# automerge/automerge-classic

Measured on AMD Instinct MI355X. Metric: CRDT ops/sec applied (bulk replay), higher is better.
Workload: dtype u32

## Files before the change

### automerge_classic_amd/csrc/am355_api.hip

```cpp
#include "am355_ctx.h"
#include "am355_scan.h"
#include "am355_textrec.h"

static bool ctx_init(am355_ctx* c) {
  {
    unsigned hw = std::thread::hardware_concurrency();
    const char* env = getenv("AM355_HOST_THREADS");
    unsigned want = env && atoi(env) > 0 ? (unsigned)atoi(env) : std::min(hw ? hw : 4u, 64u);
    c->pool.reset(new HostPool(want > 1 ? want - 1 : 0));
  }
  int prio_low = 0, prio_high = 0;
  (void)hipDeviceGetStreamPriorityRange(&prio_low, &prio_high);
  auto make_stream = [](Stream& s, int prio) { return hipStreamCreateWithPriority(&s.h, hipStreamNonBlocking, prio) == hipSuccess; };
  if (!make_stream(c->stream, prio_high)) return false;
  {
    const char* env = getenv("AM355_HASH_CUS");
    int want = env ? atoi(env) : 0;
    bool made = false;
    if (want > 0) {
      hipDeviceProp_t prop;
      if (hipGetDeviceProperties(&prop, c->device) == hipSuccess && prop.multiProcessorCount > want) {
        int n_cu = prop.multiProcessorCount;
        std::vector<uint32_t> mask((size_t)(n_cu + 31) / 32, 0u);
        for (int k = 0; k < want; k++) { int cu = n_cu - 1 - k; mask[(size_t)cu / 32] |= 1u << (cu % 32); }
// ... 9 lines not shown
  if (!c->h_sig.ensure(sizeof(HostSignals))) return false;
  memset(c->h_sig.p, 0, sizeof(HostSignals));
  if (const char* e = getenv("AM355_PHASE_EVENTS")) c->phase_events = strcmp(e, "0") != 0;
  return true;
}

extern "C" am355_ctx* am355_create(int device) {
  int n = 0;
  if (hipGetDeviceCount(&n) != hipSuccess || n <= 0 || device < 0 || device >= n) return nullptr;
  (void)hipSetDeviceFlags(hipDeviceScheduleSpin);
  if (hipSetDevice(device) != hipSuccess) return nullptr;
  am355_ctx* c = new am355_ctx();
  c->device = device;
  if (!ctx_init(c)) { delete c; return nullptr; }
  return c;
}

am355_ctx::~am355_ctx() {
  (void)hipSetDevice(device);
  if (lane) lane->wait();
  (void)doc_sum.wait();
  for (const Stream* s : {&stream, &stream2, &stream3, &stream4})
    if (s->h) (void)hipStreamSynchronize(s->h);
  if (shard_comm) (void)am355_shard_finalize(this);
}

extern "C" void am355_destroy(am355_ctx* c) {
  delete c;
}

extern "C" const char* am355_last_error(const am355_ctx* c) { return c ? c->err.c_str() : "no context (no GPU?)"; }
extern "C" uint32_t am355_flags(const am355_ctx* c) { return c ? c->flags : 0; }

extern "C" int am355_set_phase_events(am355_ctx* c, int on) {
  if (!c) return AM355_E_ARG;
  c->phase_events = on != 0;
  return AM355_OK;
}

extern "C" int am355_get_stats(const am355_ctx* c, am355_stats* out) {
  if (!c || !out) return AM355_E_ARG;
  *out = c->stats;
  return AM355_OK;
}

extern "C" int am355_get_hashes(const am355_ctx* c, uint8_t* out) {
  if (!c || !out) return AM355_E_ARG;
  if (!c->replayed || !c->h_hashes.p || c->is_document) return AM355_E_STATE;
  memcpy(out, c->h_hashes.p, 32 * (size_t)c->n_changes);
  return AM355_OK;
}

extern "C" int am355_arena_epoch(const am355_ctx* c, uint64_t* epoch) {
  if (!c || !epoch) return AM355_E_ARG;
  *epoch = c->arena_epoch;
  return AM355_OK;
}

extern "C" int am355_get_hashes_range(const am355_ctx* c, uint32_t first, uint32_t count, uint8_t* out) {
  if (!c || (!out && count)) return AM355_E_ARG;
  if (!c->replayed || !c->h_hashes.p || c->is_document) return AM355_E_STATE;
  if (first > c->n_changes || count > c->n_changes - first) return AM355_E_ARG;
  if (count) memcpy(out, (const uint8_t*)c->h_hashes.p + 32 * (size_t)first, 32 * (size_t)count);
  return AM355_OK;
}

extern "C" int am355_applied_in_input_order(const am355_ctx* c, int* yes) {
  if (!c || !yes) return AM355_E_ARG;
  if (!c->replayed || c->is_document) return AM355_E_STATE;
  bool ok = c->pending_change.empty() && c->n_pending == 0 && c->applied_change.size() == c->n_changes;
  for (uint32_t i = 0; ok && i < c->n_changes; i++) ok = c->applied_change[i] == i;
  *yes = ok ? 1 : 0;
  return AM355_OK;
}

extern "C" int am355_resident_counters(const am355_ctx* c, uint64_t out[3]) {
  if (!c || !out) return AM355_E_ARG;
  out[0] = c->n_resident_calls;
  out[1] = c->n_resident_fallbacks;
  out[2] = c->n_resorder_calls;
  return AM355_OK;
}

extern "C" int am355_resident_maps_only_calls(const am355_ctx* c, uint64_t* out) {
  if (!c || !out) return AM355_E_ARG;
  *out = c->n_maps_only_calls;
  return AM355_OK;
}

extern "C" int am355_set_resident_new_actors(am355_ctx* c, int on) {
  if (!c) return AM355_E_ARG;
  c->resident_new_actors = on != 0;
  return AM355_OK;
}

extern "C" int am355_resident_new_actor_calls(const am355_ctx* c, uint64_t out[2]) {
  if (!c || !out) return AM355_E_ARG;
  out[0] = c->n_new_actor_calls;
  out[1] = c->n_rank_rewrites;
  return AM355_OK;
}

extern "C" int am355_set_resident_map_merge(am355_ctx* c, int on) {
  if (!c) return AM355_E_ARG;
  c->resident_map_merge = on != 0;
  return AM355_OK;
}

extern "C" int am355_resident_map_merge_calls(const am355_ctx* c, uint64_t out[2]) {
  if (!c || !out) return AM355_E_ARG;
  out[0] = c->n_map_merge_calls;
  out[1] = c->n_map_merge_declined;
  return AM355_OK;
}

extern "C" int am355_set_resident_new_objects(am355_ctx* c, int on) {
  if (!c) return AM355_E_ARG;
  c->resident_new_objects = on != 0;
  return AM355_OK;
}

extern "C" int am355_resident_new_object_calls(const am355_ctx* c, uint64_t out[2]) {
  if (!c || !out) return AM355_E_ARG;
  out[0] = c->n_new_object_calls;
  out[1] = c->n_new_object_declined;
  return AM355_OK;
}

extern "C" int am355_set_resident_counters(am355_ctx* c, int on) {
  if (!c) return AM355_E_ARG;
  c->resident_counters = on != 0;
  return AM355_OK;
}

extern "C" int am355_set_local_small(am355_ctx* c, int on) {
  if (!c) return AM355_E_ARG;
  c->local_small = on != 0;
  return AM355_OK;
}

extern "C" int am355_local_small_calls(const am355_ctx* c, uint64_t out[2]) {
  if (!c || !out) return AM355_E_ARG;
  out[0] = c->n_local_small;
  out[1] = c->n_local_small_bulk;
  return AM355_OK;
}

extern "C" int am355_resident_counter_calls(const am355_ctx* c, uint64_t out[2]) {
  if (!c || !out) return AM355_E_ARG;
  out[0] = c->n_counter_calls;
  out[1] = c->n_counter_declined;
  return AM355_OK;
}

extern "C" int am355_get_raw(const am355_ctx* c, const uint8_t** arena, const uint64_t** offsets, uint32_t* n) {
  if (!c || !c->staged) return AM355_E_STATE;
  if (arena) *arena = c->raw.data();
  if (offsets) *offsets = c->raw_off.data();
  if (n) *n = c->n_changes;
  return AM355_OK;
}

extern "C" int am355_get_applied(const am355_ctx* c, uint32_t* out, uint32_t* n_applied) {
  if (!c || !n_applied) return AM355_E_ARG;
  if (!c->replayed || c->is_document) return AM355_E_STATE;
  *n_applied = (uint32_t)c->applied_change.size();
// ... 393 lines not shown
```

### automerge_classic_amd/csrc/am355_ctx.h

```cpp
#pragma once
#include "../../include/am355.h"
#include "am355_decode.h"
#include "am355_merge.h"
#include "am355_bigcol.h"
#include "am355_encode.h"
#include "am355_prims.h"
#include "am355_render.h"
#include "am355_host.h"
#include "am355_pinflate.h"
#include "am355_history.h"
#include "am355_delta.h"
#include "am355_resorder.h"
#include "am355_apply.h"
#include "am355_sync.h"
#include "am355_sched.h"
#include "am355_hist.h"
#include "am355_canary.h"

#include <zlib.h>

#include <algorithm>
#include <atomic>
#include <chrono>
#include <cstdarg>
// ... 310 lines not shown
  std::vector<uint64_t> raw_off;
  uint32_t n_changes = 0;
  DevBuf d_plan_totals;
  bool spec_launched = false;
  bool spec_large_launched = false;
  uint32_t spec_cap_ops = 0, spec_cap_preds = 0;
  uint32_t hint_ops = 0, hint_preds = 0, hint_large = 0;
  bool staged = false, replayed = false, ir_fetched = false;
  int ir_copy_enqueued = 0;
  bool prefetch_ir = false;
  bool has_unknown_cols = false;
  bool staging_in_flight = false;
  bool is_document = false;
  ChangeMeta doc_meta{};
  std::vector<uint32_t> doc_actor_rank;
  DevBuf d_arena, d_offsets, d_metas;
  uint64_t arena_epoch = 1;
  CopyRanges pending_up;
  std::vector<uint32_t> breaks_dev;
  void* breaks_dev_ptr = nullptr;
  HostBuf h_breaks_ahead;
  bool offsets_on_device = false;
  HostBuf h_metas, h_offsets, h_sig;
  uint32_t sig_seq = 0;
  Event ev_s1;
  Event ev_fills;
  Event ev_sched;
  Event ev_plan, ev_tables;
  void* counts_zeroed_at = nullptr; size_t counts_zeroed = 0;
  bool phase_events = false;
  DevBuf d_big, d_bigvals, d_ks;
  HostBuf h_biginfo;
  BigColDesc doc_cols{};
  bool doc_serial = false;
  DevBuf d_entries, d_amap_base, d_amap_prov, d_slots, d_first_idx, d_hashes, d_hash_tab, d_min_idx, d_has_dep, d_words, d_slot_rank, d_scan1, d_plan_sums, d_dep_idx, d_self_idx, d_rank_ids;
  HostBuf h_dep_idx, h_self_idx, h_amap, h_amap_base;
  HostBuf h_slots, h_hashes, h_has_dep, h_words, h_stage, h_s1;
  DevBuf d_s1;
  ChangeBrief* hp_briefs = nullptr;
  uint32_t* hp_distinct = nullptr;
  bool have_host_metas = false;
  uint32_t amap_cap = 0, slot_mask = 0, hash_mask = 0;
  bool used_fast_path = false;

  std::vector<ChangePlan> plans;
  std::vector<uint32_t> applied_change, applied_op_base;
  struct DocSum {
    static constexpr size_t PIECE = (size_t)4 << 20;
    std::thread t;
    std::unique_ptr<std::atomic<uint8_t>[]> copied;
    size_t n_pieces = 0;
    bool pending = false, ok = false;
    bool wait() {
      if (t.joinable()) t.join();
      pending = false;
      return ok;
    }
    ~DocSum() { if (t.joinable()) t.join(); }
  } doc_sum;
  std::vector<uint8_t> doc_bytes;
  std::vector<uint8_t> saved;
  HistoryOutput history;
  bool history_ok = false; uint32_t history_flags = 0;
  std::vector<std::vector<uint8_t>> inflate_scratch;
  std::vector<std::unique_ptr<PInflateJob>> pinflate_jobs;
  std::vector<uint32_t> doc_col_rows;
  std::vector<std::pair<uint32_t, std::vector<uint8_t>>> doc_chg_cols;
  std::vector<uint8_t> doc_tail;
  bool doc_other_ops_cols = false;
  DevBuf d_save, d_enc, d_encout;
  HostBuf h_encout;
  std::vector<uint32_t> amap;
  std::vector<ActorSpan> spans;
  std::vector<uint32_t> actor_tab_off;
  std::vector<std::string> actors;
  std::vector<uint32_t> clock_actor;
  std::vector<uint64_t> clock_seq;
  std::vector<uint8_t> heads;
  uint32_t n_applied = 0, n_pending = 0;
  uint64_t n_ops = 0, n_preds = 0, max_op = 0;
  DevBuf d_plans, d_amap, d_tables;
  ActorSpan* p_spans = nullptr;
  uint32_t* p_tab_off = nullptr;

  DevBuf d_cols, d_pred, d_merge, d_sort, d_ir, d_counts;
  OpCols cols{};
  MergeBufs mb{};
  PatchIR ir{};
  HostBuf h_counts;
  Counts counts{};

  HostBuf h_ir, h_rows;
  am355_patch_ir hir{};
  std::vector<uint32_t> actor_off;
  std::vector<uint8_t> actor_bytes;
  std::string json;

  am355_stats stats{};

  std::vector<uint32_t> pending_change;
  std::vector<uint32_t> pass_first_row;
  DevBuf d_delta, d_pass, d_delta_edit, d_sched, d_hist;
  HostBuf h_sched;
  bool key_unbounded = false;
  bool device_scheduled = false;
  HostBuf h_delta;
  DeltaBufs delta{};
  bool h_tables_current = false, h_tables_were_current = false;
  bool batch_list_only = false;
  void* apply_tail = nullptr;
  ApplyPatch apply;
  bool apply_ready = false;
  std::vector<uint32_t> dep_first, dep_index;
  bool dep_graph_ready = false;
  DevBuf d_sync;
  struct GraphIndex {
    uint64_t epoch = ~0ull;
    uint32_t n_staged = 0, n_applied = 0;
    std::vector<uint32_t> dep_first, dep_index;
    std::vector<uint8_t> is_applied;
    std::vector<uint32_t> table;
    std::vector<uint32_t> dpt_first, dpt_index;
    uint32_t dpt_applied = 0;
    std::vector<uint32_t> chain_head, chain_tail, chain_child, chain_next;
    std::vector<uint32_t> out_idx;
    std::vector<uint8_t> out_hashes;
    std::vector<uint64_t> absent;
    uint64_t tab_epoch = ~0ull;
    uint32_t tab_n = 0, tab_mask = 0;
  } graph;
  uint64_t graph_epoch = 0;
  uint32_t graph_probe_min = 65536;
  uint64_t n_graph_device = 0, n_graph_host = 0;
  DevBuf d_graph;
  HostBuf h_graph;
  std::vector<uint32_t> stream_breaks;
  bool breaks_exact = true, children_hazard = false, in_apply = false;
  uint32_t graph_mode = 0, doc_n_changes = 0, sched_prefix = 0;
  bool doc_head_index_known = true, sched_graph_after = true;
  bool doc_graph_known = false;
  uint64_t doc_rows = 0;
  bool doc_rows_known = false;
  bool no_history = false;
  DevBuf d_breaks;
  HostBuf h_delta_tabs;
  bool state_checked = false;
  std::string apply_json;

  struct Keep { bool want = false; uint32_t n_changes = 0; uint64_t n_ops = 0, n_preds = 0; } keep;
  uint32_t cols_cap_ops = 0, cols_cap_preds = 0;
  bool resident_valid = false;
  struct ResidentMark { uint32_t lost[8] = {}; uint32_t n_changes = 0; uint64_t n_ops = 0, n_preds = 0; } res_mark;
  uint32_t seed_list_inc = 0;
  std::vector<uint32_t> hash_index;
  uint32_t hash_index_n = 0;
  std::vector<uint32_t> res_rank_of;
  uint32_t res_rank_n = 0;
  struct ActorMemo { std::vector<uint8_t> bytes; std::vector<uint32_t> ranks; };
  std::vector<ActorMemo> res_actor_memo;
  DevBuf d_pos, d_order_alt, d_resorder;
  uint32_t* order_alt_ptr = nullptr;
  HostBuf h_resorder;
  bool pos_valid = false;
  bool ir_stale = false;
  uint64_t n_resorder_calls = 0;
  uint64_t n_maps_only_calls = 0;
// ... 148 lines not shown
```

### automerge_classic_amd/csrc/am355_decode.h

```cpp
#pragma once
#include "am355_internal.h"

namespace am355 {
struct ParseFills {
  uint32_t* p[5];
  uint64_t n_words[5];
  uint32_t value[5];
  uint32_t n;
};
void parse_changes_host(const uint8_t* arena, const uint64_t* offsets, uint32_t n_changes, ChangeMeta* metas, uint32_t* n_entries);
void launch_parse_changes(const uint8_t* arena, const uint64_t* offsets, uint32_t n_changes, ChangeMeta* metas, uint32_t* n_entries, const ParseFills& fills,
                          hipStream_t st, bool fat = false);
int change_wave_class(const ChangeMeta& m);
void launch_hash_changes(const uint8_t* arena, const uint64_t* offsets, uint32_t n, uint8_t* hashes, uint32_t* min_idx, uint32_t* hash_tab,
                         uint32_t tab_mask, uint32_t* flags, hipStream_t st);
void launch_deps_resolve(const uint8_t* arena, const ChangeMeta* metas, const uint8_t* hashes, uint32_t n, const uint32_t* hash_tab, uint32_t tab_mask,
                         const uint32_t* min_idx, uint8_t* has_dependent, uint32_t* fast_flags, uint32_t* dep_idx, uint32_t* self_idx, hipStream_t st);
void launch_actor_intern(const uint8_t* arena, ChangeMeta* metas, uint32_t n, const uint32_t* amap_base, uint32_t* amap, uint32_t amap_cap,
                         unsigned long long* slots, uint32_t slot_mask, uint32_t* first_idx, uint32_t* flags, uint32_t* fast_flags, uint32_t* distinct,
                         void* rank_ids, ChangeBrief* briefs, uint32_t* slot_rank, unsigned long long* block_sums, uint32_t* plan_words, hipStream_t st,
                         ChangeBrief* host_briefs = nullptr);
size_t rank_ids_bytes();
size_t plan_block_sums_bytes(uint32_t n);
uint32_t distinct_capacity();
void launch_plan(const ChangeBrief* briefs, uint32_t n, const uint32_t* distinct, const uint32_t* slot_rank, uint32_t slot_mask, const unsigned long long* block_sums,
                 ChangePlan* plans, ChangePlan* plans_serial, const uint32_t* words, const uint32_t* plan_words, HostSignals* sig, uint32_t seq, hipStream_t st,
                 PlanTotals* dev_totals = nullptr, uint32_t* host_s1 = nullptr);
void launch_decode_speculative(const uint8_t* arena, const ChangeMeta* metas, const ChangePlan* plans, uint32_t n_changes, const PlanTotals* totals, uint32_t cap_ops,
                               uint32_t cap_preds, uint32_t cap_distinct, const uint32_t* amap, const uint32_t* slot_rank, OpCols cols, uint32_t* flags, hipStream_t st,
                               hipStream_t aux, bool with_large, uint32_t shard_rank = 0, uint32_t shard_world = 1);
void launch_decode_planned(const uint8_t* arena, const ChangeMeta* metas, const ChangePlan* plans, const ChangePlan* plans_serial, uint32_t n_changes,
                           uint32_t n_small, uint32_t n_large, uint32_t n_serial, const uint32_t* amap, const uint32_t* slot_rank, OpCols cols, uint32_t* flags,
                           hipStream_t st, hipStream_t aux, uint32_t shard_rank = 0, uint32_t shard_world = 1);
void launch_decode_columns(const uint8_t* arena, const ChangeMeta* metas, const ChangePlan* plans, uint32_t n_small, uint32_t n_large, uint32_t n_serial,
                           const uint32_t* amap, const uint32_t* slot_rank, OpCols cols, uint32_t* flags, hipStream_t st, hipStream_t aux, uint32_t shard_rank = 0,
                           uint32_t shard_world = 1);
void launch_doc_count(const uint8_t* arena, ChangeMeta* meta, hipStream_t st);
void launch_decode_document(const uint8_t* arena, const ChangeMeta* meta, const ChangePlan* plan, const uint32_t* actor_rank, OpCols cols,
                            uint32_t* flags, hipStream_t st);
void launch_keystr_expand(const uint32_t* run_start, const uint32_t* run_off, const uint32_t* run_len, const uint32_t* n_runs, uint32_t n_rows,
                          uint32_t* key_off, uint32_t* key_len, hipStream_t st);
}
```

### automerge_classic_amd/csrc/am355_decode.hip

```cpp
#include "am355_decode.h"
#include "am355_scan.h"

#include <cstdlib>

namespace am355 {

struct __attribute__((packed)) U8B {
  uint64_t v;
};
__host__ __device__ __forceinline__ uint64_t load_u64_unaligned(const uint8_t* p) { return ((const U8B*)p)->v; }
#ifdef AM355_LDS_IS_DISTINCT
__device__ __forceinline__ uint64_t load_u64_unaligned(LdsBytes p) { return ((const __attribute__((address_space(3))) U8B*)p)->v; }
#endif

template <class P>
struct CurT {
  P p;
  uint32_t off, len;
  uint64_t win;
  uint32_t win_off;
  __host__ __device__ __forceinline__ CurT() {}
  static constexpr uint32_t WIN_EMPTY = 0xffffff00u;
  __host__ __device__ __forceinline__ CurT(P p_, uint32_t off_, uint32_t len_) : p(p_), off(off_), len(len_), win(0), win_off(WIN_EMPTY) {}
  __host__ __device__ __forceinline__ uint32_t byte_at(uint32_t o) {
// ... 987 lines not shown
  __syncthreads();
  ex[0] = ba + ia - a; ex[1] = bb + ib - b; ex[2] = bc + ic - c;
  t[0] = ta; t[1] = tb; t[2] = tc;
}

__device__ void rank_actors(const uint32_t* __restrict__ distinct, const RankId* __restrict__ rank_ids, uint32_t* __restrict__ slot_rank,
                            uint32_t* __restrict__ plan_words) {
  __shared__ unsigned long long s_id[PLAN_RANK_MAX][PLAN_ID_MAX / 8];
  __shared__ uint32_t s_len[PLAN_RANK_MAX];
  __shared__ uint32_t s_fallback;
  static_assert(PLAN_RANK_MAX % BLOCK == 0 && PLAN_RANK_MAX <= DISTINCT_CAP, "rank_actors: records per thread");
  constexpr uint32_t PER = PLAN_RANK_MAX / BLOCK;
  const uint32_t t = threadIdx.x;
  RankId rec[PER];
  uint32_t slot_of[PER];
#pragma unroll
  for (uint32_t k = 0; k < PER; k++) {
    rec[k] = rank_ids[t + k * BLOCK];
    slot_of[k] = distinct[1 + t + k * BLOCK];
  }
  const uint32_t nd = distinct[0];
  if (t == 0) s_fallback = nd > PLAN_RANK_MAX ? 1u : 0u;
  __syncthreads();
  if (nd <= PLAN_RANK_MAX) {
#pragma unroll
    for (uint32_t k = 0; k < PER; k++) {
      const uint32_t a = t + k * BLOCK;
      if (a < nd) {
        s_len[a] = rec[k].len;
        if (rec[k].len > PLAN_ID_MAX) s_fallback = 1;
        for (uint32_t wd = 0; wd < PLAN_ID_MAX / 8; wd++) s_id[a][wd] = rec[k].w[wd];
      }
    }
  }
  __syncthreads();
  if (s_fallback) { if (t == 0) plan_words[0] = 1; return; }
#pragma unroll
  for (uint32_t k = 0; k < PER; k++) {
    const uint32_t a = t + k * BLOCK;
    if (a >= nd) break;
    uint32_t rank = 0;
    const uint32_t my_len = rec[k].len;
    static_assert(PLAN_ID_MAX == 32, "rank_actors compares four 64-bit words");
    const unsigned long long m0 = rec[k].w[0], m1 = rec[k].w[1], m2 = rec[k].w[2], m3 = rec[k].w[3];
    for (uint32_t j = 0; j < nd; j++) {
      const unsigned long long x0 = s_id[j][0], x1 = s_id[j][1], x2 = s_id[j][2], x3 = s_id[j][3];
      const bool less = x0 != m0 ? x0 < m0 : x1 != m1 ? x1 < m1 : x2 != m2 ? x2 < m2 : x3 != m3 ? x3 < m3 : s_len[j] < my_len;
      rank += less ? 1u : 0u;
    }
    slot_rank[slot_of[k]] = rank;
  }
}

__global__ __launch_bounds__(WAVE) void k_actor_first(ChangeMeta* __restrict__ metas, uint32_t n, const uint32_t* __restrict__ amap_base,
                                                       const uint32_t* __restrict__ amap, uint32_t amap_cap, const uint32_t* __restrict__ first_idx,
                                                       uint32_t* __restrict__ fast_flags) {
  wave_priority_high();
  uint32_t c = blockIdx.x, lane = threadIdx.x;
  if (c >= n) return;
  ChangeMeta* m = &metas[c];
  if (m->flags) return;
  uint32_t base = amap_base[c], ne = m->n_entries;
  if ((uint64_t)base + ne > amap_cap) return;
  uint32_t mx = 0;
  for (uint32_t k = lane; k < ne; k += WAVE) {
    uint32_t f = first_idx[amap[base + k]];
    mx = f > mx ? f : mx;
  }
  for (int d = WAVE / 2; d >= 1; d >>= 1) {
    uint32_t o = __shfl_xor(mx, d);
    mx = o > mx ? o : mx;
  }
  if (lane == 0) {
    m->max_first = mx;
    if (mx > c) atomicOr(fast_flags, (uint32_t)FF_LATE_ACTOR);
  }
}

__global__ __launch_bounds__(BLOCK) void k_actor_check(const uint8_t* __restrict__ arena, ChangeMeta* __restrict__ metas, uint32_t n,
                                                       const uint32_t* __restrict__ amap_base, const uint32_t* __restrict__ amap, uint32_t amap_cap,
                                                       const uint32_t* __restrict__ first_idx, uint32_t* __restrict__ flags, uint32_t* __restrict__ fast_flags,
                                                       ChangeBrief* __restrict__ briefs, const uint32_t* __restrict__ distinct, const RankId* __restrict__ rank_ids,
                                                       uint32_t* __restrict__ slot_rank, unsigned long long* __restrict__ block_sums, uint32_t* __restrict__ plan_words,
                                                       ChangeBrief* __restrict__ host_briefs) {
  wave_priority_high();
  __shared__ unsigned long long s_scan[BLOCK / WAVE][3];
  if (blockIdx.x + 1 == gridDim.x) {
    rank_actors(distinct, rank_ids, slot_rank, plan_words);
    return;
  }
  uint32_t c = gtid();
  const bool in_range = c < n;
  ChangeBrief br{};
  if (in_range) {
    ChangeMeta* m = &metas[c];
    br.seq = m->seq;
    br.start_op = (uint32_t)m->start_op;
    br.n_ops = m->n_ops;
    br.n_preds = m->n_preds;
    br.n_entries = m->n_entries;
    br.author_slot = m->author_slot;
    br.flags_fits = m->flags;
    if (!m->flags) {
      int wc = wave_class_of(*m);
      if (wc >= 1) br.flags_fits |= 0x80000000u;
      if (wc == 2) br.flags_fits |= 0x40000000u;
      if (m->pad & 1) br.flags_fits |= 0x20000000u;
    }
    briefs[c] = br;
    if (host_briefs) host_briefs[c] = br;
  }
  const bool valid = in_range && !(br.flags_fits & 0x1fffffffu);
  const bool has = valid && br.n_ops != 0;
  const bool small = has && (br.flags_fits & 0x40000000u), large = has && !small && (br.flags_fits & 0x80000000u), serial = has && !small && !large;
  unsigned long long ex[3], t1[3], t2[3];
  block_scan3(valid ? br.n_ops : 0u, valid ? br.n_preds : 0u, valid ? br.n_entries : 0u, s_scan, ex, t1);
  block_scan3(small ? 1u : 0u, large ? 1u : 0u, serial ? 1u : 0u, s_scan, ex, t2);
  uint32_t mx_op = has ? br.start_op + br.n_ops - 1 : 0u, bad = in_range ? (br.flags_fits & 0x1fffffffu) : 0u, unknown = in_range ? (br.flags_fits & 0x20000000u) : 0u;
  for (int d = WAVE / 2; d >= 1; d >>= 1) {
    uint32_t o = __shfl_xor(mx_op, d), ob = __shfl_xor(bad, d), ou = __shfl_xor(unknown, d);
    mx_op = o > mx_op ? o : mx_op;
    bad |= ob;
    unknown |= ou;
  }
  if ((threadIdx.x & (WAVE - 1)) == 0) {
    if (mx_op) atomicMax(&plan_words[1], mx_op);
    if (bad) atomicOr(&plan_words[2], bad);
    if (unknown) atomicOr(&plan_words[3], 1u);
  }
  if (threadIdx.x == 0) {
    unsigned long long* out = block_sums + (size_t)blockIdx.x * PLAN_SUMS;
    out[0] = t1[0]; out[1] = t1[1]; out[2] = t1[2]; out[3] = t2[0]; out[4] = t2[1]; out[5] = t2[2];
  }
}

__global__ __launch_bounds__(BLOCK) void k_plan_apply(const ChangeBrief* __restrict__ briefs, uint32_t n, const uint32_t* __restrict__ slot_rank, uint32_t slot_mask,
                                                      const unsigned long long* __restrict__ block_sums, ChangePlan* __restrict__ plans,
                                                      ChangePlan* __restrict__ plans_serial, const uint32_t* __restrict__ words, const uint32_t* __restrict__ plan_words,
                                                      const uint32_t* __restrict__ distinct, HostSignals* sig, uint32_t seq, PlanTotals* __restrict__ dev_totals,
                                                      uint32_t* __restrict__ host_s1) {
  wave_priority_high();
  __shared__ unsigned long long s_scan[BLOCK / WAVE][3];
  __shared__ unsigned long long s_base[6];
  {
    unsigned long long p0 = 0, p1 = 0, p2 = 0, p3 = 0, p4 = 0, p5 = 0;
    for (uint32_t j = threadIdx.x; j < blockIdx.x; j += BLOCK) {
      const unsigned long long* q = block_sums + (size_t)j * PLAN_SUMS;
      p0 += q[0]; p1 += q[1]; p2 += q[2]; p3 += q[3]; p4 += q[4]; p5 += q[5];
    }
    unsigned long long ex[3], t1[3], t2[3];
    block_scan3(p0, p1, p2, s_scan, ex, t1);
    block_scan3(p3, p4, p5, s_scan, ex, t2);
    if (threadIdx.x == 0) { s_base[0] = t1[0]; s_base[1] = t1[1]; s_base[2] = t1[2]; s_base[3] = t2[0]; s_base[4] = t2[1]; s_base[5] = t2[2]; }
    __syncthreads();
  }
  const uint32_t c = gtid();
  const bool in_range = c < n;
  ChangeBrief br{};
  if (in_range) br = briefs[c];
  const bool valid = in_range && !(br.flags_fits & 0x1fffffffu);
  const bool has = valid && br.n_ops != 0;
  const bool small = has && (br.flags_fits & 0x40000000u), large = has && !small && (br.flags_fits & 0x80000000u), serial = has && !small && !large;
  unsigned long long e1[3], e2[3], t1[3], t2[3];
  block_scan3(valid ? br.n_ops : 0u, valid ? br.n_preds : 0u, valid ? br.n_entries : 0u, s_scan, e1, t1);
  block_scan3(small ? 1u : 0u, large ? 1u : 0u, serial ? 1u : 0u, s_scan, e2, t2);
  if (has) {
    ChangePlan pl{c, (uint32_t)(s_base[0] + e1[0]), (uint32_t)(s_base[1] + e1[1]), (uint32_t)(s_base[2] + e1[2]),
                  br.author_slot <= slot_mask ? slot_rank[br.author_slot] : 0u, br.n_entries};
    if (small) plans[(uint32_t)(s_base[3] + e2[0])] = pl;
    else if (large) plans[n - 1 - (uint32_t)(s_base[4] + e2[1])] = pl;
    else plans_serial[(uint32_t)(s_base[5] + e2[2])] = pl;
  }
  if (blockIdx.x + 1 == gridDim.x && host_s1) {
    const uint32_t nd = distinct[0] < DISTINCT_CAP ? distinct[0] : DISTINCT_CAP;
    const uint32_t* src = words;
    for (uint32_t i = threadIdx.x; i < 16; i += BLOCK) host_s1[i] = src[i];
    uint32_t* hd = host_s1 + 16;
    for (uint32_t i = threadIdx.x; i < 1 + nd; i += BLOCK) hd[i] = distinct[i];
    const unsigned long long* ids = (const unsigned long long*)(distinct + 2 + DISTINCT_CAP);
    unsigned long long* hids = (unsigned long long*)(hd + 2 + DISTINCT_CAP);
    for (uint32_t i = threadIdx.x; i < nd; i += BLOCK) hids[i] = ids[i];
    __threadfence_system();
    __syncthreads();
  }
  if (blockIdx.x + 1 == gridDim.x && threadIdx.x == 0) {
    unsigned long long ops = s_base[0] + t1[0], preds = s_base[1] + t1[1], ent = s_base[2] + t1[2];
    PlanTotals z{};
    z.n_ops = (uint32_t)ops; z.n_preds = (uint32_t)preds; z.n_entries = (uint32_t)ent;
    z.n_small = (uint32_t)(s_base[3] + t2[0]); z.n_large = (uint32_t)(s_base[4] + t2[1]); z.n_serial = (uint32_t)(s_base[5] + t2[2]);
    z.max_op = plan_words[1];
    z.fallback = (plan_words[0] || ops >= 0x7ffffff0ull || preds >= 0xfffffff0ull || ent >= 0xfffffff0ull) ? 1u : 0u;
    z.flags_a = words[0] | plan_words[2]; z.fast_a = words[1]; z.total_entries = words[2]; z.n_distinct = distinct[0];
    z.reserved[0] = plan_words[3];
    if (dev_totals) *dev_totals = z;
    signal_host((uint32_t*)&sig->plan, (const uint32_t*)&z, sizeof(PlanTotals) / 4, &sig->plan_seq, seq);
  }
}

struct Rle {
  Cur c;
  int state;
  int64_t count;
  bool have_last, last_null;
  int64_t last;
  uint32_t last_off, last_len;
};

__device__ __forceinline__ void rle_init(Rle& r, const uint8_t* p, uint32_t len) {
  r.c = Cur(p, 0, len);
  r.state = 0;
  r.count = 0;
  r.have_last = false;
  r.last_null = true;
  r.last = 0;
  r.last_off = r.last_len = 0;
}

enum { RT_UINT = 0, RT_INT = 1, RT_UTF8 = 2 };

struct RVal {
  bool is_null;
  int64_t i;
  uint32_t off, len;
};

template <int TYPE>
__device__ __forceinline__ bool rle_raw(Rle& r, RVal& v) {
  v.is_null = false;
  if (TYPE == RT_UINT) {
    uint64_t u;
    if (!read_uleb(r.c, u)) return false;
    v.i = (int64_t)u;
  } else if (TYPE == RT_INT) {
    if (!read_sleb(r.c, v.i)) return false;
  } else {
    uint64_t n;
    if (!read_uleb(r.c, n)) return false;
    v.off = r.c.off;
    v.len = (uint32_t)n;
    if (!skip_bytes(r.c, n)) return false;
  }
  return true;
}

template <int TYPE>
__device__ __forceinline__ bool rle_same(const Rle& r, const RVal& v) {
  if (!r.have_last || r.last_null) return false;
  if (TYPE == RT_UTF8) {
    return r.last_len == v.len && bytes_equal(r.c.p, r.last_off, v.off, v.len, r.c.len);
  }
  return r.last == v.i;
}

template <int TYPE>
__device__ __forceinline__ void rle_set_last(Rle& r, const RVal& v) {
  r.have_last = true;
  r.last_null = v.is_null;
  r.last = v.i;
  r.last_off = v.off;
  r.last_len = v.len;
}

template <int TYPE>
__device__ bool rle_next(Rle& r, RVal& v) {
  if (r.count == 0 && r.c.off >= r.c.len) {
    v.is_null = true;
    v.i = 0;
    v.off = v.len = 0;
    return true;
  }
  if (r.count == 0) {
    int64_t n;
    if (!read_sleb(r.c, n)) return false;
    if (n > 1) {
      RVal x;
      x.off = x.len = 0;
// ... 853 lines not shown
      }
    }
  }
  }
  if (groups & DG_PRED) {
  uint32_t total_preds = 0;
  load_col(C_PRED_NUM);
  err |= L.err;
  {
    int64_t carry = 0;
    for (uint32_t i0 = 0; i0 < n; i0 += WAVE) {
      uint32_t i = i0 + lane;
      bool nul = true; int64_t k = 0;
      if (i < n) wv_row_value<false>(L, i, nul, k, err);
      if (nul) k = 0;
      int64_t incl = carry + wave_incl_scan_i64(k, lane);
      carry = __shfl(incl, WAVE - 1);
      if (i < n) {
        if ((uint64_t)incl > n_preds_cap) { err |= F_BAD_RLE; k = 0; incl = 0; }
        o.pred_num[base + i] = (uint32_t)k;
        o.pred_first[base + i] = pl.pred_base + (uint32_t)(incl - k);
      }
    }
    total_preds = (uint64_t)carry > n_preds_cap ? 0 : (uint32_t)carry;
  }
  load_col(C_PRED_ACTOR);
  err |= L.err;
  for (uint32_t j = lane; j < total_preds; j += WAVE) {
    bool nul; int64_t v;
    wv_row_value<false>(L, j, nul, v, err);
    uint32_t r = 0;
    if (nul) err |= F_UNSUPPORTED;
    else if ((uint64_t)v >= pl.n_actors) err |= F_BAD_ROW;
    else r = L.rank[v];
    o.pred_actor[pl.pred_base + j] = r;
  }
  load_col(C_PRED_CTR);
  err |= L.err;
  {
    int64_t carry = 0;
    for (uint32_t j0 = 0; j0 < total_preds; j0 += WAVE) {
      uint32_t j = j0 + lane;
      bool nul = true; int64_t d = 0;
      if (j < total_preds) wv_row_value<true>(L, j, nul, d, err);
      int64_t abs = carry + wave_incl_scan_i64(nul ? 0 : d, lane);
      carry = __shfl(abs, WAVE - 1);
      if (j < total_preds) {
        if (nul) err |= F_UNSUPPORTED;
        else if (abs < 0 || (uint64_t)abs >= NONE32) err |= F_OVERFLOW;
        o.pred_ctr[pl.pred_base + j] = (uint32_t)abs;
      }
    }
  }
  }
  if (err) atomicOr(flags, err);
}

int change_wave_class(const ChangeMeta& m) { return wave_class_of(m); }

void launch_parse_changes(const uint8_t* arena, const uint64_t* offsets, uint32_t n_changes, ChangeMeta* metas, uint32_t* n_entries, const ParseFills& fills,
                          hipStream_t st, bool fat) {
  if (!n_changes && !fills.n) return;
  if (fat) hipLaunchKernelGGL(k_parse_changes<true>, dim3(n_changes ? n_changes : 64), dim3(WAVE), 0, st, arena, offsets, n_changes, metas, n_entries, fills);
  else hipLaunchKernelGGL(k_parse_changes<false>, dim3(n_changes ? n_changes : 64), dim3(WAVE), 0, st, arena, offsets, n_changes, metas, n_entries, fills);
}

void launch_hash_changes(const uint8_t* arena, const uint64_t* offsets, uint32_t n, uint8_t* hashes, uint32_t* min_idx, uint32_t* hash_tab,
                         uint32_t tab_mask, uint32_t* flags, hipStream_t st) {
  if (!n) return;
  hipLaunchKernelGGL(k_hash_changes, dim3((n + HASH_LANES - 1) / HASH_LANES), dim3(2 * HASH_LANES), 0, st, arena, offsets, n, hashes, min_idx, flags);
  AM355_LAUNCH_INDEPENDENT(k_hash_insert, dim3((n + BLOCK - 1) / BLOCK), dim3(BLOCK), st, (const uint8_t*)hashes, n, hash_tab, tab_mask, min_idx);
}

void launch_deps_resolve(const uint8_t* arena, const ChangeMeta* metas, const uint8_t* hashes, uint32_t n, const uint32_t* hash_tab, uint32_t tab_mask,
                         const uint32_t* min_idx, uint8_t* has_dependent, uint32_t* fast_flags, uint32_t* dep_idx, uint32_t* self_idx, hipStream_t st) {
  if (!n) return;
  AM355_LAUNCH_INDEPENDENT(k_deps_resolve, dim3(n), dim3(WAVE), st, arena, metas, hashes, n, hash_tab, tab_mask, min_idx, has_dependent, fast_flags, dep_idx,
                           self_idx);
}

void launch_actor_intern(const uint8_t* arena, ChangeMeta* metas, uint32_t n, const uint32_t* amap_base, uint32_t* amap, uint32_t amap_cap,
                         unsigned long long* slots, uint32_t slot_mask, uint32_t* first_idx, uint32_t* flags, uint32_t* fast_flags, uint32_t* distinct,
                         void* rank_ids, ChangeBrief* briefs, uint32_t* slot_rank, unsigned long long* block_sums, uint32_t* plan_words, hipStream_t st,
                         ChangeBrief* host_briefs) {
  if (n)
    hipLaunchKernelGGL(k_actor_intern, dim3(n), dim3(WAVE), 0, st, arena, metas, n, amap_base, amap, amap_cap, slots, slot_mask, first_idx, flags,
                       fast_flags, distinct, (RankId*)rank_ids);
  if (n) hipLaunchKernelGGL(k_actor_first, dim3(n), dim3(WAVE), 0, st, metas, n, amap_base, (const uint32_t*)amap, amap_cap, (const uint32_t*)first_idx, fast_flags);
  hipLaunchKernelGGL(k_actor_check, dim3((n + BLOCK - 1) / BLOCK + 1), dim3(BLOCK), 0, st, arena, metas, n, amap_base, (const uint32_t*)amap, amap_cap,
                     (const uint32_t*)first_idx, flags, fast_flags, briefs, (const uint32_t*)distinct, (const RankId*)rank_ids, slot_rank, block_sums, plan_words,
                     host_briefs);
}

size_t rank_ids_bytes() { return sizeof(RankId) * PLAN_RANK_MAX; }

size_t plan_block_sums_bytes(uint32_t n) { return sizeof(unsigned long long) * PLAN_SUMS * ((size_t)(n + BLOCK - 1) / BLOCK + 1); }

void launch_plan(const ChangeBrief* briefs, uint32_t n, const uint32_t* distinct, const uint32_t* slot_rank, uint32_t slot_mask, const unsigned long long* block_sums,
                 ChangePlan* plans, ChangePlan* plans_serial, const uint32_t* words, const uint32_t* plan_words, HostSignals* sig, uint32_t seq, hipStream_t st,
                 PlanTotals* dev_totals, uint32_t* host_s1) {
  uint32_t nb = (n + BLOCK - 1) / BLOCK;
  hipLaunchKernelGGL(k_plan_apply, dim3(nb ? nb : 1), dim3(BLOCK), 0, st, briefs, n, slot_rank, slot_mask, block_sums, plans, plans_serial, words, plan_words,
                     distinct, sig, seq, dev_totals, host_s1);
}

uint32_t distinct_capacity() { return DISTINCT_CAP; }

__global__ __launch_bounds__(WAVE) void k_doc_count(const uint8_t* __restrict__ arena, ChangeMeta* __restrict__ meta) {
  uint32_t lane = threadIdx.x;
  if (lane > 1) return;
  int slot = lane == 0 ? C_ACTION : C_PRED_NUM;
  uint64_t cnt, sum;
  bool ok = rle_count_sum(arena + meta->base + meta->col_off[slot], meta->col_len[slot], cnt, sum);
  if (!ok) { atomicOr(&meta->flags, (uint32_t)F_BAD_RLE); return; }
  if (lane == 0) meta->n_ops = (uint32_t)cnt; else meta->n_preds = (uint32_t)sum;
}

void launch_doc_count(const uint8_t* arena, ChangeMeta* meta, hipStream_t st) {
  AM355_LAUNCH_INDEPENDENT(k_doc_count, dim3(1), dim3(WAVE), st, arena, meta);
}

__global__ __launch_bounds__(BLOCK) void k_keystr_expand(const uint32_t* __restrict__ run_start, const uint32_t* __restrict__ run_off,
                                                          const uint32_t* __restrict__ run_len, const uint32_t* __restrict__ n_runs_p, uint32_t n_rows,
                                                          uint32_t* __restrict__ key_off, uint32_t* __restrict__ key_len) {
  uint32_t row = gtid();
  if (row >= n_rows) return;
  uint32_t nr = *n_runs_p;
  uint32_t off = 0, len = NONE32;
  if (nr && row < run_start[nr]) {
    uint32_t lo = 0, hi = nr;
    while (hi - lo > 1) {
      uint32_t mid = (lo + hi) >> 1;
      if (run_start[mid] <= row) lo = mid; else hi = mid;
    }
    off = run_off[lo];
    len = run_len[lo];
  }
  key_off[row] = off;
  key_len[row] = len;
}

void launch_keystr_expand(const uint32_t* run_start, const uint32_t* run_off, const uint32_t* run_len, const uint32_t* n_runs, uint32_t n_rows,
                          uint32_t* key_off, uint32_t* key_len, hipStream_t st) {
  if (!n_rows) return;
  AM355_LAUNCH_INDEPENDENT(k_keystr_expand, dim3((n_rows + BLOCK - 1) / BLOCK), dim3(BLOCK), st, run_start, run_off, run_len, n_runs, n_rows, key_off, key_len);
}

void launch_decode_document(const uint8_t* arena, const ChangeMeta* meta, const ChangePlan* plan, const uint32_t* actor_rank, OpCols cols,
                            uint32_t* flags, hipStream_t st) {
  ActorXlate x{actor_rank, nullptr, 0, 1};
  AM355_LAUNCH_INDEPENDENT(k_decode_columns, dim3(1, T_NUM_DOC), dim3(WAVE), st, arena, meta, plan, 1u, x, cols, flags, 0);
}

static uint32_t decode_group_split(uint32_t n_waves, uint32_t shard_world, bool large_class = false) {
  static const uint32_t split_max = []() { const char* e = getenv("AM355_DECODE_SPLIT_MAX"); return e && atol(e) > 0 ? (uint32_t)atol(e) : 1536u; }();
  return (shard_world <= 1 && n_waves <= (large_class ? 512u : split_max)) ? 4u : 1u;
}

void launch_decode_columns(const uint8_t* arena, const ChangeMeta* metas, const ChangePlan* plans, uint32_t n_small, uint32_t n_large, uint32_t n_serial,
                           const uint32_t* amap, const uint32_t* slot_rank, OpCols cols, uint32_t* flags, hipStream_t st, hipStream_t aux, uint32_t shard_rank,
                           uint32_t shard_world) {
  ActorXlate x{amap, slot_rank, shard_rank, shard_world};
  if (n_large && n_small + n_large <= 1024) { n_large += n_small; n_small = 0; }
  hipStream_t s2 = (n_small && aux) ? aux : st;
  if (n_small) hipLaunchKernelGGL(k_decode_wave<WaveLdsSmall>, dim3(n_small, decode_group_split(n_small, shard_world)), dim3(WAVE), 0, st, arena, metas, plans, n_small, x, cols, flags, DecodeGate{});
  if (n_large) hipLaunchKernelGGL(k_decode_wave<WaveLdsLarge>, dim3(n_large, decode_group_split(n_large, shard_world, true)), dim3(WAVE), 0, s2, arena, metas, plans + n_small, n_large, x, cols, flags, DecodeGate{});
  if (n_serial)
    AM355_LAUNCH_INDEPENDENT(k_decode_columns, dim3((n_serial + WAVE - 1) / WAVE, T_NUM), dim3(WAVE), s2, arena, metas, plans + n_small + n_large, n_serial,
                             x, cols, flags, 0);
}

void launch_decode_planned(const uint8_t* arena, const ChangeMeta* metas, const ChangePlan* plans, const ChangePlan* plans_serial, uint32_t n_changes,
                           uint32_t n_small, uint32_t n_large, uint32_t n_serial, const uint32_t* amap, const uint32_t* slot_rank, OpCols cols, uint32_t* flags,
                           hipStream_t st, hipStream_t aux, uint32_t shard_rank, uint32_t shard_world) {
  ActorXlate x{amap, slot_rank, shard_rank, shard_world};
  hipStream_t s2 = (n_small && aux) ? aux : st;
  if (n_small) hipLaunchKernelGGL(k_decode_wave<WaveLdsSmall>, dim3(n_small, decode_group_split(n_small, shard_world)), dim3(WAVE), 0, st, arena, metas, plans, n_small, x, cols, flags, DecodeGate{});
  if (n_large) hipLaunchKernelGGL(k_decode_wave<WaveLdsLarge>, dim3(n_large, decode_group_split(n_large, shard_world, true)), dim3(WAVE), 0, s2, arena, metas, plans + (n_changes - n_large), n_large, x, cols, flags, DecodeGate{});
  if (n_serial)
    AM355_LAUNCH_INDEPENDENT(k_decode_columns, dim3((n_serial + WAVE - 1) / WAVE, T_NUM), dim3(WAVE), s2, arena, metas, plans_serial, n_serial, x, cols, flags, 0);
}

void launch_decode_speculative(const uint8_t* arena, const ChangeMeta* metas, const ChangePlan* plans, uint32_t n_changes, const PlanTotals* totals, uint32_t cap_ops,
                               uint32_t cap_preds, uint32_t cap_distinct, const uint32_t* amap, const uint32_t* slot_rank, OpCols cols, uint32_t* flags, hipStream_t st,
                               hipStream_t aux, bool with_large, uint32_t shard_rank, uint32_t shard_world) {
  if (!n_changes) return;
  ActorXlate x{amap, slot_rank, shard_rank, shard_world};
  hipLaunchKernelGGL(k_decode_wave<WaveLdsSmall>, dim3(n_changes, decode_group_split(n_changes, shard_world)), dim3(WAVE), 0, st, arena, metas, plans, 0u, x, cols, flags,
                     DecodeGate{totals, cap_ops, cap_preds, cap_distinct, n_changes, 0u});
// ... 7 lines not shown
```

### automerge_classic_amd/csrc/am355_replay.hip

```cpp
#include "am355_ctx.h"


template <class IsHead>
static void set_heads(am355_ctx* c, uint32_t n, IsHead is_head) {
  std::vector<const uint8_t*> hs;
  for (uint32_t i = 0; i < n; i++)
    if (is_head(i)) hs.push_back(c->h_hashes.as<uint8_t>() + 32 * (size_t)i);
  std::sort(hs.begin(), hs.end(), [](const uint8_t* x, const uint8_t* y) { return memcmp(x, y, 32) < 0; });
  c->heads.resize(hs.size() * 32);
  for (size_t i = 0; i < hs.size(); i++) memcpy(&c->heads[32 * i], hs[i], 32);
}

template <class SpanOf>
static int build_actor_spans(am355_ctx* c, uint32_t na, std::vector<uint32_t>& cnt, SpanOf span_of) {
  c->actor_tab_off.assign(na + 1, 0);
  for (uint32_t a = 0; a < na; a++) c->actor_tab_off[a + 1] = c->actor_tab_off[a] + cnt[a];
  c->spans.resize(c->actor_tab_off[na]);
  for (uint32_t a = 0; a < na; a++) cnt[a] = c->actor_tab_off[a];
  for (const ChangePlan& pl : c->plans) { ActorSpan s = span_of(pl); s.op_base = pl.op_base; c->spans[cnt[pl.author]++] = s; }
  for (uint32_t a = 0; a < na; a++) {
    ActorSpan* v = c->spans.data() + c->actor_tab_off[a];
    size_t k_n = c->actor_tab_off[a + 1] - c->actor_tab_off[a];
    bool sorted = true;
    for (size_t k = 1; k < k_n; k++) sorted = sorted && v[k - 1].start_op <= v[k].start_op;
    if (!sorted) std::sort(v, v + k_n, [](const ActorSpan& x, const ActorSpan& y) { return x.start_op < y.start_op; });
    for (size_t k = 1; k < k_n; k++)
      if ((uint64_t)v[k - 1].start_op + v[k - 1].n_ops > v[k].start_op) {
        c->flags |= AM355_F_DUP_OPID;
        return fail(c, AM355_E_INVALID, "overlapping op id ranges for one actor (duplicate operation ID)");
      }
  }
  return AM355_OK;
}

static constexpr uint32_t UNSET = 0xffffffffu, NEVER = 0xfffffffeu, BUSY = 0xfffffffdu;

struct LineageInput {
  uint32_t n, na, na0, nd;
  bool doc_head_index_known;
  const ChangeMeta* metas;
  const uint32_t *self, *dep_idx, *dep_first, *dep_count, *rank, *local_ids, *local_off;
  std::vector<uint8_t> doc_has_dependent;
};
struct LineageOutcome { std::vector<uint32_t> pass, gpass, gpos; bool graph_after = true; uint32_t flags = 0; };
static LineageOutcome schedule_lineage(const LineageInput& in, bool graph_known) {
  const uint32_t n = in.n, na0 = in.na0, nd = in.nd;
  const ChangeMeta* metas = in.metas;
  LineageOutcome o;
  auto author_of = [&](uint32_t ci) { return in.rank[in.local_ids[in.local_off[ci]]]; };
  auto group_of = [&](uint32_t ci) { return in.self[ci] < n ? in.self[ci] : ci; };
  o.pass.assign(n, NEVER); o.gpass.assign(n, NEVER); o.gpos.assign(n, 0);
  std::vector<uint8_t> vis_dep(n, 0), vis_dup(n, 0), in_round(n, 0);
  std::vector<uint64_t> clk(in.na, 0);
  for (uint32_t i = 0; i < na0; i++) { clk[author_of(i)] = metas[i].seq; o.pass[i] = 0; o.gpass[group_of(i)] = 0; o.gpos[group_of(i)] = i; }
  auto all_prior = [&]() {
    std::fill(vis_dep.begin(), vis_dep.end(), 0); std::fill(vis_dup.begin(), vis_dup.end(), 0);
    for (uint32_t i = 0; i < na0; i++) vis_dep[group_of(i)] = vis_dup[group_of(i)] = 1;
  };
  if (graph_known) all_prior();
  else {
    for (uint32_t i = nd; i < na0; i++) vis_dep[group_of(i)] = vis_dup[group_of(i)] = 1;
    for (uint32_t i = 0; i < nd; i++)
      if (!in.doc_has_dependent[i]) { vis_dup[i] = 1; vis_dep[i] = in.doc_head_index_known ? 1 : 0; }
  }
  std::vector<uint32_t> queue, app, enq;
  for (uint32_t ci = na0; ci < n; ci++) queue.push_back(ci);
  bool graph = graph_known;
  uint32_t round_pass = 0;
  while (!queue.empty()) {
    app.clear(); enq.clear();
    std::vector<uint64_t> clk2 = clk;
    bool aborted = false;
    for (uint32_t ci : queue) {
      const uint32_t F = group_of(ci);
      if (vis_dup[F] || in_round[F]) continue;
      bool ready = true;
      for (uint32_t k = 0; k < in.dep_count[ci] && ready; k++) { const uint32_t dd = in.dep_idx[in.dep_first[ci] + k]; ready = dd < n && (vis_dep[dd] || in_round[dd]); }
      const uint32_t a = author_of(ci);
      const uint64_t expected = clk2[a] + 1;
      if (!ready) enq.push_back(ci);
      else if (metas[ci].seq < expected) {
        if (graph) { o.flags |= AM355_F_BAD_SEQ; return o; }
        aborted = true;
        break;
      } else if (metas[ci].seq > expected) { o.flags |= AM355_F_BAD_SEQ; return o; }
      else { clk2[a] = metas[ci].seq; in_round[F] = 1; app.push_back(ci); }
    }
    for (uint32_t ci : app) in_round[group_of(ci)] = 0;
    if (aborted) { app.clear(); enq = queue; }
    if (!app.empty()) {
      for (uint32_t ci : app) { const uint32_t F = group_of(ci); o.pass[ci] = round_pass; o.gpass[F] = round_pass; o.gpos[F] = ci; vis_dep[F] = vis_dup[F] = 1; }
      clk = clk2;
      round_pass++;
    }
    queue = enq;
    if (queue.empty()) break;
    if (app.empty()) {
      if (graph) break;
      graph = true;
      all_prior();
    }
  }
  o.graph_after = graph;
  return o;
}

static uint32_t rank_device_actors(am355_ctx* c, std::vector<uint32_t>& slot_rank);
// ... 195 lines not shown
  uint64_t ops = 0, preds = 0, max_op = 0;
  std::vector<uint32_t> span_cnt(na + 1, 0);
  c->applied_change.clear();
  c->applied_op_base.clear();
  c->pass_first_row.clear();
  for (size_t t = 0; t < applied_all.size(); t++) {
    uint32_t ci = applied_all[t];
    const ChangeMeta& m = metas[ci];
    if (t > 0 && applied_pass[t] != applied_pass[t - 1]) c->pass_first_row.push_back((uint32_t)ops);
    c->applied_change.push_back(ci);
    c->applied_op_base.push_back((uint32_t)ops);
    ChangePlan pl;
    pl.change = ci;
    pl.op_base = (uint32_t)ops;
    pl.pred_base = (uint32_t)preds;
    pl.amap_base = (uint32_t)c->amap.size();
    pl.author = rank[local_ids[local_off[ci]]];
    pl.n_actors = local_off[ci + 1] - local_off[ci];
    for (uint32_t k = local_off[ci]; k < local_off[ci + 1]; k++) c->amap.push_back(rank[local_ids[k]]);
    if (m.n_ops) {
      span_cnt[pl.author]++;
      max_op = std::max<uint64_t>(max_op, m.start_op + m.n_ops - 1);
      c->plans.push_back(pl);
    }
    ops += m.n_ops;
    preds += m.n_preds;
    if (ops >= 0x7ffffff0ull || preds >= 0xfffffff0ull) { c->flags |= AM355_F_OVERFLOW; return fail(c, AM355_E_UNSUPPORTED, "more than 2^31 ops in one batch"); }
  }
  c->n_ops = ops;
  c->n_preds = preds;
  c->max_op = max_op;
  { int src = build_actor_spans(c, na, span_cnt, [&](const ChangePlan& pl) { return ActorSpan{(uint32_t)metas[pl.change].start_op, metas[pl.change].n_ops, 0}; }); if (src) return src; }
  if (getenv("AM355_DEBUG_TIMING")) {
    auto T4 = std::chrono::steady_clock::now();
    auto ms = [](auto a, auto b) { return std::chrono::duration<double, std::milli>(b - a).count(); };
    fprintf(stderr, "schedule: actors %.3f rank %.3f causal %.3f plan %.3f ms\n", ms(T0, T1), ms(T1, T2), ms(T2, T3), ms(T3, T4));
  }
  return AM355_OK;
}


static uint32_t rank_device_actors(am355_ctx* c, std::vector<uint32_t>& slot_rank) {
  const uint32_t* distinct = c->hp_distinct;
  const unsigned long long* slots = (const unsigned long long*)(distinct + 2 + distinct_capacity());
  const uint8_t* raw = c->raw.data();
  uint32_t n_slots = c->slot_mask + 1;
  struct Ent { uint32_t slot, off, len; };
  static thread_local std::vector<Ent> ents;
  ents.clear();
  uint32_t nd = distinct[0];
  for (uint32_t k = 0; k < nd; k++) {
    uint32_t i = distinct[1 + k];
    ents.push_back(Ent{i, (uint32_t)((slots[k] >> 16) - 1), (uint32_t)(slots[k] & 0xffff)});
  }
  std::sort(ents.begin(), ents.end(), [&](const Ent& x, const Ent& y) {
    uint32_t m = std::min(x.len, y.len);
    int r = m ? memcmp(raw + x.off, raw + y.off, m) : 0;
    return r ? r < 0 : x.len < y.len;
  });
  uint32_t na = (uint32_t)ents.size();
  slot_rank.assign(n_slots, 0);
  c->actors.resize(na);
  for (uint32_t r = 0; r < na; r++) {
    slot_rank[ents[r].slot] = r;
    c->actors[r].assign((const char*)raw + ents[r].off, ents[r].len);
  }
  return na;
}

static int plan_fast(am355_ctx* c, std::vector<uint32_t>& slot_rank, const uint32_t* order = nullptr, uint32_t n_applied = 0, const uint32_t* pass = nullptr) {
  const ChangeBrief* br = c->hp_briefs;
  uint32_t n = order ? n_applied : c->n_changes;
  uint32_t na = rank_device_actors(c, slot_rank);
  static thread_local std::vector<uint64_t> clock;
  static thread_local std::vector<uint32_t> span_cnt;
  clock.assign(na, 0);
  span_cnt.assign(na + 1, 0);
  c->clock_actor.clear();
  c->plans.clear();
  c->plans.reserve(n);
  c->applied_change.resize(n);
  c->applied_op_base.resize(n);
  c->pass_first_row.clear();
  uint64_t ops = 0, preds = 0, entries = 0, max_op = 0;
  for (uint32_t t = 0; t < n; t++) {
    const uint32_t ci = order ? order[t] : t;
    const ChangeBrief& m = br[ci];
    if (order && t > 0 && pass[ci] != pass[order[t - 1]]) c->pass_first_row.push_back((uint32_t)ops);
    c->applied_change[t] = ci;
    c->applied_op_base[t] = (uint32_t)ops;
    uint32_t author = slot_rank[m.author_slot];
    if (m.seq != clock[author] + 1) { c->flags |= AM355_F_BAD_SEQ; return fail(c, AM355_E_INVALID, "sequence number %llu out of order", (unsigned long long)m.seq); }
    if (clock[author] == 0) c->clock_actor.push_back(author);
    clock[author] = m.seq;
    if (m.n_ops) {
      c->plans.push_back(ChangePlan{ci, (uint32_t)ops, (uint32_t)preds, (uint32_t)entries, author, m.n_entries});
      span_cnt[author]++;
      max_op = std::max<uint64_t>(max_op, (uint64_t)m.start_op + m.n_ops - 1);
    }
    ops += m.n_ops;
    preds += m.n_preds;
    entries += m.n_entries;
    if (ops >= 0x7ffffff0ull || preds >= 0xfffffff0ull) { c->flags |= AM355_F_OVERFLOW; return fail(c, AM355_E_UNSUPPORTED, "more than 2^31 ops in one batch"); }
  }
  c->n_applied = n;
  c->n_pending = 0;
  c->pending_change.clear();
  c->n_ops = ops;
  c->n_preds = preds;
  c->max_op = max_op;
  c->clock_seq.clear();
  for (uint32_t a : c->clock_actor) c->clock_seq.push_back(clock[a]);
  return build_actor_spans(c, na, span_cnt, [&](const ChangePlan& pl) { return ActorSpan{br[pl.change].start_op, br[pl.change].n_ops, 0}; });
}

static int carve_cols(am355_ctx* c, uint32_t N, uint32_t P, bool estimate = false) {
  canary_scope("replay buffers (carve_cols: op rows, preds)");
  if (c->in_apply && !estimate) {
    N = (uint32_t)std::min<uint64_t>((uint64_t)N + N / 4 + 65536, 0x7ffffff0u);
    P = (uint32_t)std::min<uint64_t>((uint64_t)P + P / 4 + 65536, 0xfffffff0u);
  }
  c->cols_cap_ops = N;
  c->cols_cap_preds = P;
  c->resident_valid = false;
  size_t Nc = (size_t)N + 1;
  size_t bytes = 13 * carve_size(Nc, 4) + carve_size(Nc, 1);
  if (!c->d_cols.ensure(bytes) || !c->d_pred.ensure(2 * carve_size((size_t)P + 1, 4))) return fail(c, AM355_E_NOMEM, "device allocation failed (op rows)");
  canary_forget(c->d_cols.p, c->d_cols.cap); canary_forget(c->d_pred.p, c->d_pred.cap);
  uint8_t* p = c->d_cols.as<uint8_t>();
  OpCols& o = c->cols;
  o.obj_actor = carve<uint32_t>(p, Nc); o.obj_ctr = carve<uint32_t>(p, Nc); o.key_actor = carve<uint32_t>(p, Nc); o.key_ctr = carve<uint32_t>(p, Nc);
  o.key_off = carve<uint32_t>(p, Nc); o.key_len = carve<uint32_t>(p, Nc); o.action = carve<uint32_t>(p, Nc); o.val_tl = carve<uint32_t>(p, Nc);
  o.val_off = carve<uint32_t>(p, Nc); o.pred_first = carve<uint32_t>(p, Nc); o.pred_num = carve<uint32_t>(p, Nc); o.id_ctr = carve<uint32_t>(p, Nc);
  o.id_actor = carve<uint32_t>(p, Nc); o.insert = carve<uint8_t>(p, Nc);
  uint8_t* q = c->d_pred.as<uint8_t>();
  o.pred_actor = carve<uint32_t>(q, (size_t)P + 1);
  o.pred_ctr = carve<uint32_t>(q, (size_t)P + 1);
  return AM355_OK;
}

int setup_buffers(am355_ctx* c, uint32_t NA) {
  uint32_t N = (uint32_t)c->n_ops, P = (uint32_t)c->n_preds;
  int bits_ctr = bits_for64(c->max_op), bits_actor = bits_for64(NA ? NA - 1 : 0), bits_row = bits_for64(N);
  if (1 + bits_row + bits_ctr + bits_actor > 64) { c->flags |= AM355_F_OVERFLOW; return fail(c, AM355_E_UNSUPPORTED, "sort key wider than 64 bits"); }
  size_t Nc = (size_t)N + 1;
  c->resident_valid = false;
  c->order_alt_ptr = nullptr;
  c->map_alt_ptr = nullptr;
  c->pos_valid = false;
  c->ir_stale = false;
  canary_scope("replay buffers (setup_buffers: op rows, preds, merge scratch, sort scratch, patch IR)");
  if (!(c->spec_launched && N <= c->spec_cap_ops && P <= c->spec_cap_preds)) {
    c->spec_launched = false;
    int rcc = carve_cols(c, N, P);
    if (rcc) return rcc;
  }
  canary_scope("replay buffers (setup_buffers: merge scratch, sort scratch, patch IR)");
  const bool by_cap = c->in_apply && c->cols_cap_ops >= N;
  if (by_cap) Nc = std::min<size_t>(c->cols_cap_ops, (size_t)N + N / 4 + 65536) + 1;
  {
    size_t cw = carry_words((uint32_t)(Nc - 1));
    size_t bytes = 10 * carve_size(Nc, 4) + 3 * carve_size(Nc, 8) + carve_size(Nc, 1) + carve_size(2 * Nc + 2, 4) + 4 * carve_size(2 * Nc + 2, 4) +
                   3 * carve_size(Nc + 1, 4) + scan_workspace_bytes((uint32_t)(2 * Nc + 2)) + 256 +
                   6 * carve_size(Nc + 3, 4) + 6 * carve_size(cw, 4) + carve_size(2048, 4);
    size_t sort_bytes = 2 * carve_size(Nc, 8) + 2 * carve_size(Nc, 4) + sort_workspace_bytes((uint32_t)Nc) + 256;
    size_t ir_bytes = carve_size(Nc + 1, sizeof(am355_ir_object)) + carve_size(Nc, sizeof(am355_ir_map)) + carve_size(Nc + 1, sizeof(am355_ir_edit)) +
                      4 * carve_size(Nc, 4);
    if (!c->d_merge.ensure(bytes) || !c->d_sort.ensure(sort_bytes) || !c->d_ir.ensure(ir_bytes) || !c->d_counts.ensure(merge_counts_bytes(N)))
      return fail(c, AM355_E_NOMEM, "device allocation failed (merge)");
    canary_forget(c->d_merge.p, c->d_merge.cap); canary_forget(c->d_sort.p, c->d_sort.cap); canary_forget(c->d_ir.p, c->d_ir.cap);
    uint8_t* p = c->d_merge.as<uint8_t>();
    MergeBufs& b = c->mb;
    b.arena = c->d_arena.as<uint8_t>();
    b.ops = c->cols;
    b.n_ops = N; b.n_preds = P; b.n_actors = NA;
    b.shard_rank = c->shard_rank; b.shard_world = c->shard_world;
    b.sig = c->h_sig.as<HostSignals>(); b.sig_seq = c->sig_seq;
    b.actor_tab_off = c->p_tab_off;
    b.spans = c->p_spans;
    b.bits_ctr = (uint32_t)bits_ctr; b.bits_actor = (uint32_t)bits_actor;
    b.first_row = 0; b.seed_list_inc = 0; b.row_stride = by_cap ? (uint32_t)Nc : 0u;
    b.zero_base = p;
    b.succ_cnt = carve<uint32_t>(p, Nc); b.inc_cnt = carve<uint32_t>(p, Nc); b.val_cnt = carve<uint32_t>(p, Nc);
    b.inc_sum = carve<unsigned long long>(p, Nc); b.last_inc = carve<unsigned long long>(p, Nc);
    b.zero_bytes = (size_t)(p - (uint8_t*)b.zero_base) - (canary_on() ? 256 : 0);
    canary_allow(b.zero_base, b.zero_bytes);
    b.obj_row = carve<uint32_t>(p, Nc); b.ref_row = carve<uint32_t>(p, Nc); b.obj_index = carve<uint32_t>(p, Nc);
    b.em_row = carve<uint32_t>(p, Nc); b.ins_row = carve<uint32_t>(p, Nc); b.upd_row = carve<uint32_t>(p, Nc); b.next_sib = carve<uint32_t>(p, Nc);
    b.em_trig = carve<unsigned long long>(p, Nc);
    b.kind = carve<uint8_t>(p, Nc);
    b.order = carve<uint32_t>(p, Nc + 1);
    b.first_child = carve<uint32_t>(p, 2 * Nc + 2);
    b.euler_b = carve<unsigned long long>(p, 2 * Nc + 2); b.euler_a = carve<unsigned long long>(p, 2 * Nc + 2);
    b.scan_a = carve<uint32_t>(p, Nc + 1); b.scan_b = carve<uint32_t>(p, Nc + 1);
    b.scan_ws = p;
    canary_note(p, scan_workspace_bytes((uint32_t)(2 * Nc + 2)));
    p += carve_round(scan_workspace_bytes((uint32_t)(2 * Nc + 2)));
    b.run_heads = carve<uint32_t>(p, Nc + 3); b.row_run = carve<uint32_t>(p, Nc + 3); b.obj_n = carve<uint32_t>(p, Nc + 3);
    b.obj_first_pos = carve<uint32_t>(p, Nc + 3); b.list_vis = carve<uint32_t>(p, Nc + 3); b.list_cnt = carve<uint32_t>(p, Nc + 3);
    b.cs_ins.wg_sum = carve<uint32_t>(p, cw); b.cs_make.wg_sum = carve<uint32_t>(p, cw); b.cs_runs.wg_sum = carve<uint32_t>(p, cw);
    b.cs_vis.wg_sum = carve<uint32_t>(p, cw); b.cs_cnt.wg_sum = carve<uint32_t>(p, cw); b.cs_erec.wg_sum = carve<uint32_t>(p, cw);
    b.head_child = carve<uint32_t>(p, 2048);
    b.child_head = (uint32_t*)b.euler_b;
    b.child_next = b.child_head + (2 * Nc + 2);
    b.fill_base = b.order;
    b.fill_bytes = (size_t)((uint8_t*)(b.child_head + 2 * Nc + 1) - (uint8_t*)b.order);
    canary_allow(b.fill_base, b.fill_bytes);
    uint8_t* s = c->d_sort.as<uint8_t>();
    b.key_a = carve<uint64_t>(s, Nc); b.key_b = carve<uint64_t>(s, Nc); b.val_a = carve<uint32_t>(s, Nc); b.val_b = carve<uint32_t>(s, Nc);
    b.sort_ws = s;
    merge_bind_counts(b, c->d_counts.p);
    uint8_t* r = c->d_ir.as<uint8_t>();
    PatchIR& ir = c->ir;
    ir.obj = carve<am355_ir_object>(r, Nc + 1); ir.map = carve<am355_ir_map>(r, Nc); ir.edit = carve<am355_ir_edit>(r, Nc + 1);
    ir.e_row = carve<uint32_t>(r, Nc); ir.e_elem = carve<uint32_t>(r, Nc); ir.e_index = carve<uint32_t>(r, Nc); ir.e_flags = carve<uint32_t>(r, Nc);
  }
  canary_arm();
  return AM355_OK;
}

static void take_counts(am355_ctx* c, const Counts* hc) { c->counts = *hc; c->counts.n_objects += 1; }

static int merge_and_take_counts(am355_ctx* c) {
  Counts* hc = c->h_counts.as<Counts>();
  merge_run(c->mb, c->ir, hc, c->stream, (c->phase_events || !c->mb.sig) ? c->ev_counts.h : nullptr, c->ev_runs);
  HIPCHK(c, hipEventRecord(c->ev[5], c->stream));
  if (hc->flags) return error_for_flags(c, hc->flags, "op set rejected");
  take_counts(c, hc);
  return AM355_OK;
}

static void fill_stats_of_state(am355_ctx* c) {
  am355_stats& s = c->stats;
  s.n_changes = c->n_changes; s.n_applied = c->n_applied; s.n_pending = c->n_pending; s.n_actors = (uint32_t)c->actors.size(); s.n_objects = c->counts.n_objects;
  s.n_heads = (uint32_t)(c->heads.size() / 32); s.n_ops = c->n_ops; s.max_op = c->max_op; s.raw_bytes = c->raw.size();
  s.n_map_values = c->counts.n_map_emit; s.n_list_elems = c->counts.n_list_ins; s.n_edits = c->counts.n_edits;
  s.ir_bytes = (uint64_t)c->counts.n_objects * sizeof(am355_ir_object) + (uint64_t)c->counts.n_map_emit * sizeof(am355_ir_map) +
               ((uint64_t)c->counts.n_erecs + 1) * sizeof(am355_ir_edit);
}

static int run_device(am355_ctx* c, const std::vector<uint32_t>* slot_rank) {
  hipStream_t st = c->stream;
  size_t np = c->plans.size();
  auto al = [](size_t b) { return (b + 255) & ~(size_t)255; };
  size_t b_plans = sizeof(ChangePlan) * np, b_spans = sizeof(ActorSpan) * c->spans.size(), b_tab = 4 * c->actor_tab_off.size();
  size_t b_rank = slot_rank ? 4 * slot_rank->size() : 0, b_amap = slot_rank ? 0 : 4 * c->amap.size();
  size_t o_spans = al(b_plans + 16), o_tab = o_spans + al(b_spans + 16), o_x = o_tab + al(b_tab + 16), tables_bytes = o_x + al(std::max(b_rank, b_amap) + 16);
  if (!c->d_tables.ensure(tables_bytes) || !c->h_stage.ensure(tables_bytes)) return fail(c, AM355_E_NOMEM, "device allocation failed");
  uint8_t* d_tables = c->d_tables.as<uint8_t>();
  c->p_spans = (ActorSpan*)(d_tables + o_spans);
  c->p_tab_off = (uint32_t*)(d_tables + o_tab);
  c->sig_seq++;
  int rcb = setup_buffers(c, (uint32_t)c->actors.size());
  if (rcb) return rcb;
  uint32_t n_small = 0, n_large = 0;
  {
    const ChangeBrief* br = c->hp_briefs;
    std::vector<ChangePlan> large, serial;
    size_t w = 0;
    for (size_t i = 0; i < np; i++) {
      uint32_t f = br[c->plans[i].change].flags_fits;
      if (f & 0x40000000u) c->plans[w++] = c->plans[i];
      else if (f & 0x80000000u) large.push_back(c->plans[i]);
      else serial.push_back(c->plans[i]);
    }
    n_small = (uint32_t)w;
    n_large = (uint32_t)large.size();
    for (auto& pl : large) c->plans[w++] = pl;
    for (auto& pl : serial) c->plans[w++] = pl;
  }
  const uint32_t* d_amap;
  const uint32_t* d_rank = nullptr;
  {
    uint8_t* h = c->h_stage.as<uint8_t>();
    if (b_plans) memcpy(h, c->plans.data(), b_plans);
    if (b_spans) memcpy(h + o_spans, c->spans.data(), b_spans);
    if (b_tab) memcpy(h + o_tab, c->actor_tab_off.data(), b_tab);
    if (slot_rank) {
      if (b_rank) memcpy(h + o_x, slot_rank->data(), b_rank);
      d_amap = c->d_amap_prov.as<uint32_t>();
      d_rank = (const uint32_t*)(d_tables + o_x);
    } else {
      if (b_amap) memcpy(h + o_x, c->amap.data(), b_amap);
      d_amap = (const uint32_t*)(d_tables + o_x);
    }
    HIPCHK(c, hipMemcpyAsync(d_tables, h, o_x + std::max(b_rank, b_amap), hipMemcpyHostToDevice, st));
  }

  HIPCHK(c, hipMemsetAsync(c->d_counts.p, 0, c->mb.counts_bytes, st));
  HIPCHK(c, hipEventRecord(c->ev_fork, st));
  HIPCHK(c, hipStreamWaitEvent(c->stream3, c->ev_fork, 0));
  if (!merge_prepare(c->mb, c->stream3)) return fail(c, AM355_E_DEVICE, "merge fills: more ranges than one launch takes");
  HIPCHK(c, hipEventRecord(c->ev[2], st));
  launch_decode_columns(c->d_arena.as<uint8_t>(), c->d_metas.as<ChangeMeta>(), (const ChangePlan*)d_tables, n_small, n_large, (uint32_t)np - n_small - n_large, d_amap,
                        d_rank, c->cols, &c->d_counts.as<Counts>()->flags, st, c->stream3, c->shard_rank, c->shard_world);
  HIPCHK(c, hipEventRecord(c->ev[3], st));
  HIPCHK(c, hipEventRecord(c->ev_join, c->stream3));
  HIPCHK(c, hipStreamWaitEvent(st, c->ev_join, 0));
  return merge_and_take_counts(c);
}

struct GeneralOrder { const uint32_t* order; const uint32_t* pass; uint32_t n_applied; hipEvent_t ready; };
static int run_device_planned(am355_ctx* c, const PlanTotals& tot, uint32_t n_distinct, float* ms_host_plan, const GeneralOrder* go = nullptr) {
  hipStream_t st = c->stream;
  const TraceLap lap("  planned:", 26);
  const bool trace = lap.on;
  uint32_t n = c->n_changes;
  c->n_ops = tot.n_ops;
  c->n_preds = tot.n_preds;
  c->max_op = tot.max_op;
  auto al = [](size_t b) { return (b + 255) & ~(size_t)255; };
  size_t o_tab = al(sizeof(ActorSpan) * (size_t)n + 16), tables_bytes = o_tab + al(4 * ((size_t)n_distinct + 1) + 16);
  if (!c->d_tables.ensure(tables_bytes) || !c->h_stage.ensure(tables_bytes)) return fail(c, AM355_E_NOMEM, "device allocation failed");
  uint8_t* d_tables = c->d_tables.as<uint8_t>();
  c->p_spans = (ActorSpan*)d_tables;
  c->p_tab_off = (uint32_t*)(d_tables + o_tab);
  c->sig_seq++;
  int rcb = setup_buffers(c, n_distinct);
  if (rcb) return rcb;
  lap("buffers carved");
  const bool spec_done = c->spec_launched && decode_gate_open(tot, c->spec_cap_ops, c->spec_cap_preds, distinct_capacity()) &&
                         c->counts_zeroed_at == c->d_counts.p && c->mb.counts_bytes <= c->counts_zeroed;
  if (trace && c->spec_launched && !spec_done)
    fprintf(stderr, "  planned: speculative decode not usable: ops %u / cap %u, preds %u / cap %u, distinct %u, fast_a %x flags_a %x fallback %u, counts %p/%p %zu/%zu\n", tot.n_ops,
            c->spec_cap_ops, tot.n_preds, c->spec_cap_preds, tot.n_distinct, tot.fast_a, tot.flags_a, tot.fallback, c->counts_zeroed_at, c->d_counts.p, c->mb.counts_bytes, c->counts_zeroed);
  if (c->spec_launched && !spec_done) {
    c->spec_launched = false;
    HIPCHK(c, hipStreamSynchronize(c->stream3));
    HIPCHK(c, hipStreamSynchronize(st));
    int rc2 = setup_buffers(c, n_distinct);
    if (rc2) return rc2;
  }
  if (!spec_done && !(c->counts_zeroed_at == c->d_counts.p && c->mb.counts_bytes <= c->counts_zeroed)) HIPCHK(c, hipMemsetAsync(c->d_counts.p, 0, c->mb.counts_bytes, st));
  c->counts_zeroed_at = nullptr;
  c->hint_large = tot.n_large;
  if (spec_done) {
    c->hint_ops = std::max(c->hint_ops, tot.n_ops);
    c->hint_preds = std::max(c->hint_preds, tot.n_preds);
    const uint32_t host_large = c->spec_large_launched ? 0u : tot.n_large;
    if (tot.n_serial || host_large) {
      if (!c->spec_large_launched) {
        HIPCHK(c, hipEventRecord(c->ev_fork, st));
        HIPCHK(c, hipStreamWaitEvent(c->stream3, c->ev_fork, 0));
      }
      launch_decode_planned(c->d_arena.as<uint8_t>(), c->d_metas.as<ChangeMeta>(), c->d_plans.as<ChangePlan>(), c->d_plans.as<ChangePlan>() + std::max(n, 1u), n, 0,
                            host_large, tot.n_serial, c->d_amap_prov.as<uint32_t>(), c->d_slot_rank.as<uint32_t>(), c->cols, &c->d_counts.as<Counts>()->flags,
                            c->stream3, nullptr, c->shard_rank, c->shard_world);
    }
    lap("decode was launched behind the plan kernel");
  } else {
    c->hint_ops = tot.n_ops;
    c->hint_preds = tot.n_preds;
    if (tot.n_small && (tot.n_large || tot.n_serial)) {
      HIPCHK(c, hipEventRecord(c->ev_fork, st));
      HIPCHK(c, hipStreamWaitEvent(c->stream3, c->ev_fork, 0));
    }
    if (c->phase_events) HIPCHK(c, hipEventRecord(c->ev[2], st));
    launch_decode_planned(c->d_arena.as<uint8_t>(), c->d_metas.as<ChangeMeta>(), c->d_plans.as<ChangePlan>(), c->d_plans.as<ChangePlan>() + std::max(n, 1u), n,
                          tot.n_small, tot.n_large, tot.n_serial, c->d_amap_prov.as<uint32_t>(), c->d_slot_rank.as<uint32_t>(), c->cols,
                          &c->d_counts.as<Counts>()->flags, st, c->stream3, c->shard_rank, c->shard_world);
    lap("decode launched");
    if (c->phase_events) HIPCHK(c, hipEventRecord(c->ev[3], st));
  }
  c->spec_launched = false;
  const bool second_class = tot.n_small && (tot.n_large || tot.n_serial);
  hipStream_t fill_stream = second_class ? c->stream4 : c->stream3;
  if (!merge_prepare(c->mb, fill_stream)) return fail(c, AM355_E_DEVICE, "merge fills: more ranges than one launch takes");
  if (second_class) {
    HIPCHK(c, hipEventRecord(c->ev_join, c->stream3));
    HIPCHK(c, hipStreamWaitEvent(st, c->ev_join, 0));
  }
  lap("fills enqueued");
  if (go) HIPCHK(c, hipEventSynchronize(go->ready));
  auto t0 = std::chrono::steady_clock::now();
  std::vector<uint32_t> slot_rank;
  int rc = go ? plan_fast(c, slot_rank, go->order, go->n_applied, go->pass) : plan_fast(c, slot_rank);
  *ms_host_plan = std::chrono::duration<float, std::milli>(std::chrono::steady_clock::now() - t0).count();
  lap("plan_fast done");
  if (rc == AM355_OK && (c->n_ops != tot.n_ops || c->n_preds != tot.n_preds || c->max_op != tot.max_op || c->actors.size() != n_distinct))
    rc = fail(c, AM355_E_DEVICE, "internal: device and host plans disagree (%llu / %u ops)", (unsigned long long)c->n_ops, tot.n_ops);
  if (rc) { (void)hipStreamSynchronize(st); return rc; }
  {
    uint8_t* h = c->h_stage.as<uint8_t>();
    size_t b_spans = sizeof(ActorSpan) * c->spans.size(), b_tab = 4 * c->actor_tab_off.size();
    if (b_spans) memcpy(h, c->spans.data(), b_spans);
    memcpy(h + o_tab, c->actor_tab_off.data(), b_tab);
    HIPCHK(c, hipMemcpyAsync(d_tables, h, o_tab + b_tab, hipMemcpyHostToDevice, fill_stream));
    HIPCHK(c, hipEventRecord(c->ev_tables, fill_stream));
    HIPCHK(c, hipStreamWaitEvent(st, c->ev_tables, 0));
  }
  lap("tables enqueued");
  return merge_and_take_counts(c);
}

static int replay_document_stages(am355_ctx* c) {
  auto t_begin = std::chrono::steady_clock::now();
  const TraceLap lap("replay_document:", 28, t_begin);
  hipStream_t st = c->stream;
  uint32_t NA = (uint32_t)c->actors.size();
  if (!c->d_plans.ensure(sizeof(ChangePlan)) || !c->d_amap.ensure(4 * (size_t)std::max(NA, 1u)) || !c->d_words.ensure(4 * W_NUM) || !c->h_words.ensure(4 * W_NUM))
    return fail(c, AM355_E_NOMEM, "device allocation failed");
  HIPCHK(c, hipEventRecord(c->ev[0], st));
  c->doc_col_rows.clear();
  if (c->doc_serial) {
    HIPCHK(c, hipMemcpyAsync(c->d_metas.p, &c->doc_meta, sizeof(ChangeMeta), hipMemcpyHostToDevice, st));
    launch_doc_count(c->d_arena.as<uint8_t>(), c->d_metas.as<ChangeMeta>(), st);
    HIPCHK(c, hipMemcpyAsync(c->h_metas.p, c->d_metas.p, sizeof(ChangeMeta), hipMemcpyDeviceToHost, st));
    HIPCHK(c, hipEventRecord(c->ev[1], st));
    HIPCHK(c, hipStreamSynchronize(st));
    const ChangeMeta* hm = c->h_metas.as<ChangeMeta>();
    if (hm->flags) return error_for_flags(c, hm->flags, "malformed document columns");
    c->n_ops = hm->n_ops;
    c->n_preds = hm->n_preds;
    c->n_applied = c->n_changes;
    c->n_pending = 0;
    c->max_op = 0xffffffffu >> 8;
    if (c->n_ops >= 0x7ffffff0ull) { c->flags |= AM355_F_OVERFLOW; return fail(c, AM355_E_UNSUPPORTED, "more than 2^31 rows in one document"); }
    int rc = setup_buffers(c, NA);
    if (rc) return rc;
    ChangePlan pl{0, 0, 0, 0, NONE32, NA};
    HIPCHK(c, hipMemcpyAsync(c->d_plans.p, &pl, sizeof pl, hipMemcpyHostToDevice, st));
    HIPCHK(c, hipMemcpyAsync(c->d_amap.p, c->doc_actor_rank.data(), 4 * (size_t)NA, hipMemcpyHostToDevice, st));
    HIPCHK(c, hipMemsetAsync(c->d_counts.p, 0, c->mb.counts_bytes, st));
    HIPCHK(c, hipMemsetAsync(c->d_words.p, 0, 4 * W_NUM, st));
    HIPCHK(c, hipEventRecord(c->ev[2], st));
    launch_decode_document(c->d_arena.as<uint8_t>(), c->d_metas.as<ChangeMeta>(), c->d_plans.as<ChangePlan>(), c->d_amap.as<uint32_t>(), c->cols,
                           &c->d_counts.as<Counts>()->flags, st);
  } else {
    const BigColDesc& d = c->doc_cols;
    const ChangeMeta& m = c->doc_meta;
    if (!c->d_big.ensure(bigcol_work_bytes(d.tok_bytes)) || !c->d_ks.ensure(keystr_work_bytes(m.col_len[C_KEY_STR])) || !c->h_biginfo.ensure(sizeof(BigColInfo)))
      return fail(c, AM355_E_NOMEM, "device allocation failed (document index)");
    BigColWork w;
    canary_forget(c->d_big.p, c->d_big.cap);
    bigcol_carve(w, c->d_big.p, d.tok_bytes);
    canary_arm();
    uint32_t *ks_start, *ks_off, *ks_len;
    uint32_t* d_words = c->d_words.as<uint32_t>();
    HIPCHK(c, hipMemsetAsync(d_words, 0, 4 * W_NUM, st));
    HIPCHK(c, hipMemcpyAsync(c->d_amap.p, c->doc_actor_rank.data(), 4 * (size_t)NA, hipMemcpyHostToDevice, st));
    lap("actor ranks enqueued");
    HIPCHK(c, hipEventRecord(c->ev_b0, st));
    HIPCHK(c, hipStreamWaitEvent(c->stream2, c->ev_b0, 0));
    KeyStage ks;
    ks.max_jumps = c->key_unbounded ? 0u : 64u;
    canary_forget(c->d_ks.p, c->d_ks.cap);
    keystr_index_begin(c->d_arena.as<uint8_t>(), m.col_off[C_KEY_STR], m.col_len[C_KEY_STR], c->d_ks.p, ks, d_words + W_TOTAL_ENTRIES, d_words + W_FAST_B,
                       c->stream2);
    keystr_index_finish(ks, false, &ks_start, &ks_off, &ks_len, d_words + W_FLAGS_B, c->stream2);
    HIPCHK(c, hipEventRecord(c->ev_b1, c->stream2));
    lap("key stream enqueued");
    BigColInfo* hi = c->h_biginfo.as<BigColInfo>();
    bigcol_index_tokens(c->d_arena.as<uint8_t>(), d, w, st);
    HIPCHK(c, hipMemcpyAsync(hi, w.info, sizeof(BigColInfo), hipMemcpyDeviceToHost, st));
    lap("token ends enqueued");
    HIPCHK(c, hipStreamSynchronize(st));
    bigcol_index_records(c->d_arena.as<uint8_t>(), d, w, hi->n_tokens, st);
    HIPCHK(c, hipMemcpyAsync(hi, w.info, sizeof(BigColInfo), hipMemcpyDeviceToHost, st));
    HIPCHK(c, hipEventRecord(c->ev[1], st));
    lap("enqueued index");
    HIPCHK(c, hipStreamSynchronize(st));
    lap("token index done");
    if (hi->flags) { (void)hipStreamSynchronize(c->stream2); return error_for_flags(c, hi->flags, "malformed document columns"); }
    BigColInfo info = *hi;
// ... 892 lines not shown
                      ((uint64_t)c->counts.n_erecs + 1) * sizeof(am355_ir_edit);
  if (verify) {
    std::vector<uint32_t> now(c->counts.n_list_ins);
    HIPCHK(c, hipMemcpy(now.data(), b.order, 4 * now.size(), hipMemcpyDeviceToHost));
    if (now != kept) return fail(c, AM355_E_DEVICE, "internal: the list order merged in place differs from the order computed from scratch");
    const size_t NO = c->counts.n_objects;
    if (NO != kept_obj.size())
      return fail(c, AM355_E_DEVICE, "internal: %zu objects kept from the in-place calls, %zu computed from scratch", kept_obj.size(), NO);
    std::vector<am355_ir_object> obj(NO);
    std::vector<uint32_t> first(NO), cnt(NO);
    if (NO) {
      HIPCHK(c, hipMemcpy(obj.data(), c->ir.obj, sizeof(am355_ir_object) * NO, hipMemcpyDeviceToHost));
      HIPCHK(c, hipMemcpy(first.data(), b.obj_first_pos, 4 * NO, hipMemcpyDeviceToHost));
      HIPCHK(c, hipMemcpy(cnt.data(), b.obj_n, 4 * NO, hipMemcpyDeviceToHost));
    }
    for (size_t k = 1; k < NO; k++) {
      const am355_ir_object &x = kept_obj[k], &y = obj[k];
      if (x.id_ctr != y.id_ctr || x.id_actor != y.id_actor || x.type != y.type || x.make_row != y.make_row)
        return fail(c, AM355_E_DEVICE, "internal: object %zu kept from the in-place calls is %u@%u type %u row %u, computed from scratch %u@%u type %u row %u", k,
                    x.id_ctr, x.id_actor, x.type, x.make_row, y.id_ctr, y.id_actor, y.type, y.make_row);
    }
    for (size_t k = 0; k < NO; k++)
      if (kept_first[k] != first[k] || kept_n[k] != cnt[k])
        return fail(c, AM355_E_DEVICE, "internal: object %zu kept from the in-place calls has %u elements from position %u, computed from scratch %u from %u", k,
                    kept_n[k], kept_first[k], cnt[k], first[k]);
  }
  return AM355_OK;
}

static constexpr size_t S1_DISTINCT = 64;

struct Stage1 {
  uint32_t n = 0;
  size_t n1 = 1;
  uint32_t *d_wa = nullptr, *d_distinct = nullptr;
  ChangeBrief* d_briefs = nullptr;
  uint32_t *d_words = nullptr, *h_words = nullptr;
  HostSignals* sig = nullptr;
  size_t counts_bytes = 0;
  bool counts_cleared = false, fat_changes = false;
  bool hash_enqueued = false, spec_possible = false;
  PlanTotals tot{};
  bool fast = false, planned = false, lineage_schedule = false;
  std::chrono::steady_clock::time_point t_host0;
  float ms_host = 0;
  int opt_rc = AM355_OK;
  uint32_t opt_flags = 0;
  std::string opt_err;
  std::atomic<int> lane_rc{AM355_OK};
  LaneJoin lane_join;
};

static int replay_on_resident_state(am355_ctx* c, std::chrono::steady_clock::time_point t_begin) {
  const int rr = replay_resident(c);
  if (rr != AM355_OK) return rr;
  am355_stats& s = c->stats;
  fill_stats_of_state(c);
  s.ms_parse = s.ms_decode = s.ms_merge = s.ms_order = s.ms_hash_stream = s.ms_host_schedule = 0;
  s.fast_path = 1;
  s.ms_total = std::chrono::duration<float, std::milli>(std::chrono::steady_clock::now() - t_begin).count();
  c->used_fast_path = true;
  c->device_scheduled = false;
  c->replayed = true;
  c->seed_list_inc = c->counts.n_list_inc;
  resident_mark(c);
  c->resident_valid = true;
  return AM355_OK;
}

static int replay_stage1_buffers(am355_ctx* c, Stage1& s) {
  const uint32_t n = s.n = c->n_changes;
  const size_t n1 = s.n1 = std::max<size_t>(n, 1);
  c->slot_mask = pow2_at_least(4 * (uint64_t)n + 64) - 1;
  c->hash_mask = pow2_at_least(2 * (uint64_t)n + 64) - 1;
  if (c->amap_cap < 16 * n1 + 1024) c->amap_cap = (uint32_t)(16 * n1 + 1024);
  if (!c->d_entries.ensure(4 * n1) || !c->d_amap_base.ensure(4 * (n1 + 1)) || !c->d_amap_prov.ensure(4 * (size_t)c->amap_cap) ||
      !c->d_slots.ensure(8 * (size_t)(c->slot_mask + 1)) || !c->d_first_idx.ensure(4 * (size_t)(c->slot_mask + 1)) || !c->d_hashes.ensure(32 * n1) ||
      !c->d_hash_tab.ensure(4 * (size_t)(c->hash_mask + 1)) || !c->d_min_idx.ensure(4 * n1) || !c->d_has_dep.ensure(n1) || !c->d_words.ensure(4 * W_NUM) ||
      !c->d_scan1.ensure(scan_workspace_bytes((uint32_t)n1)) || !c->h_slots.ensure(8 * (size_t)(c->slot_mask + 1)) || !c->h_hashes.ensure(32 * n1) ||
      !c->h_has_dep.ensure(n1) || !c->h_words.ensure(4 * W_NUM) || !c->d_plans.ensure(2 * sizeof(ChangePlan) * n1) ||
      !c->d_slot_rank.ensure(4 * (size_t)(c->slot_mask + 1)) || !c->d_plan_sums.ensure(plan_block_sums_bytes(n)) ||
      !c->d_dep_idx.ensure(4 * (c->raw.size() / 32 + 2)) || !c->d_self_idx.ensure(4 * n1) || !c->d_rank_ids.ensure(rank_ids_bytes()))
    return fail(c, AM355_E_NOMEM, "device allocation failed (stage 1)");
  c->have_host_metas = false;
  const size_t s1_briefs = S1_DISTINCT + ((12 * (size_t)distinct_capacity() + 16 + 63) & ~(size_t)63);
  const size_t s1_bytes = s1_briefs + sizeof(ChangeBrief) * n1;
  if (!c->d_s1.ensure(s1_bytes) || !c->h_s1.ensure(s1_bytes)) return fail(c, AM355_E_NOMEM, "device allocation failed (stage 1)");
  s.d_wa = c->d_s1.as<uint32_t>();
  s.d_distinct = (uint32_t*)(c->d_s1.as<uint8_t>() + S1_DISTINCT);
  s.d_briefs = (ChangeBrief*)(c->d_s1.as<uint8_t>() + s1_briefs);
  c->hp_distinct = (uint32_t*)(c->h_s1.as<uint8_t>() + S1_DISTINCT);
  c->hp_briefs = (ChangeBrief*)(c->h_s1.as<uint8_t>() + s1_briefs);
  s.d_words = c->d_words.as<uint32_t>();
  s.h_words = c->h_words.as<uint32_t>();
  s.sig = c->h_sig.as<HostSignals>();
  return AM355_OK;
}

static int replay_parse(am355_ctx* c, Stage1& s) {
  hipStream_t sa = c->stream;
  HIPCHK(c, hipEventRecord(c->ev[0], sa));
  s.counts_bytes = merge_counts_bytes((uint32_t)std::min<size_t>(c->raw.size(), 0x7ffffff0u));
  c->counts_zeroed_at = nullptr;
  s.counts_cleared = c->d_counts.ensure(s.counts_bytes);
  s.fat_changes = s.n && c->raw.size() / s.n > 4096 && !getenv("AM355_PARSE_LEAN");
  ParseFills f{};
  auto add = [&](void* q, size_t bytes, uint32_t v) { f.p[f.n] = (uint32_t*)q; f.n_words[f.n] = (bytes + 3) / 4; f.value[f.n] = v; f.n++; };
  add(s.d_words, 4 * W_NUM, 0);
  add(s.d_wa, S1_DISTINCT + 16, 0);
  add(c->d_slots.p, 8 * (size_t)(c->slot_mask + 1), 0);
  add(c->d_first_idx.p, 4 * (size_t)(c->slot_mask + 1), 0xffffffffu);
  if (s.counts_cleared) add(c->d_counts.p, s.counts_bytes, 0);
  launch_parse_changes(c->d_arena.as<uint8_t>(), c->d_offsets.as<uint64_t>(), s.n, c->d_metas.as<ChangeMeta>(), c->d_entries.as<uint32_t>(), f, sa, s.fat_changes);
  HIPCHK(c, hipEventRecord(c->ev_parse, sa));
  if (s.counts_cleared) {
    c->counts_zeroed_at = c->d_counts.p;
    c->counts_zeroed = s.counts_bytes;
  }
  return AM355_OK;
}

static int replay_enqueue_hash_stream(am355_ctx* c, const Stage1& s) {
  hipStream_t sb = c->stream2;
  const uint32_t n = s.n;
  HIPCHK(c, hipStreamWaitEvent(sb, c->ev_parse, 0));
  HIPCHK(c, hipEventRecord(c->ev_b0, sb));
  HIPCHK(c, hipMemsetAsync(c->d_hash_tab.p, 0, 4 * (size_t)(c->hash_mask + 1), sb));
  HIPCHK(c, hipMemsetAsync(c->d_has_dep.p, 0, s.n1, sb));
  launch_hash_changes(c->d_arena.as<uint8_t>(), c->d_offsets.as<uint64_t>(), n, c->d_hashes.as<uint8_t>(), c->d_min_idx.as<uint32_t>(),
                  c->d_hash_tab.as<uint32_t>(), c->hash_mask, s.d_words + W_FLAGS_B, sb);
  launch_deps_resolve(c->d_arena.as<uint8_t>(), c->d_metas.as<ChangeMeta>(), c->d_hashes.as<uint8_t>(), n, c->d_hash_tab.as<uint32_t>(), c->hash_mask,
                  c->d_min_idx.as<uint32_t>(), c->d_has_dep.as<uint8_t>(), s.d_words + W_FAST_B, c->d_dep_idx.as<uint32_t>(), c->d_self_idx.as<uint32_t>(), sb);
  HIPCHK(c, hipMemcpyAsync(c->h_hashes.p, c->d_hashes.p, 32 * (size_t)n, hipMemcpyDeviceToHost, sb));
  HIPCHK(c, hipMemcpyAsync(c->h_has_dep.p, c->d_has_dep.p, n, hipMemcpyDeviceToHost, sb));
  HIPCHK(c, hipMemcpyAsync(s.h_words + W_FLAGS_B, s.d_words + W_FLAGS_B, 8, hipMemcpyDeviceToHost, sb));
  HIPCHK(c, hipEventRecord(c->ev_b1, sb));
  return AM355_OK;
}

static void replay_post_hash_stream(am355_ctx* c, Stage1& s) {
  if (!(AM355_STREAMS_ORDER_ACROSS_THREADS && s.n >= 512)) return;
  if (!c->lane) c->lane.reset(new AsyncLane);
  c->lane->post([c, &s]() { (void)hipSetDevice(c->device); s.lane_rc.store(replay_enqueue_hash_stream(c, s)); });
  s.lane_join.l = c->lane.get();
  s.hash_enqueued = true;
}

static int replay_intern_and_plan(am355_ctx* c, Stage1& s, const TraceLap& lap) {
  hipStream_t sa = c->stream;
  const uint32_t n = s.n;
  exclusive_scan_u32(c->d_entries.as<uint32_t>(), c->d_amap_base.as<uint32_t>(), n, s.d_wa + W_TOTAL_ENTRIES, c->d_scan1.p, sa);
  s.spec_possible = n && s.counts_cleared && !getenv("AM355_HOST_PLAN") && !(c->in_apply && c->graph_mode != 0) && c->d_plan_totals.ensure(sizeof(PlanTotals));
  for (int attempt = 0;; attempt++) {
    if (attempt) {
      HIPCHK(c, hipMemsetAsync(c->d_slots.p, 0, 8 * (size_t)(c->slot_mask + 1), sa));
      HIPCHK(c, hipMemsetAsync(c->d_first_idx.p, 0xff, 4 * (size_t)(c->slot_mask + 1), sa));
      HIPCHK(c, hipMemsetAsync(s.d_distinct, 0, 4, sa));
    }
    launch_actor_intern(c->d_arena.as<uint8_t>(), c->d_metas.as<ChangeMeta>(), n, c->d_amap_base.as<uint32_t>(), c->d_amap_prov.as<uint32_t>(), c->amap_cap,
                        c->d_slots.as<unsigned long long>(), c->slot_mask, c->d_first_idx.as<uint32_t>(), s.d_wa + W_FLAGS_A, s.d_wa + W_FAST_A,
                        s.d_distinct, c->d_rank_ids.p, s.d_briefs, c->d_slot_rank.as<uint32_t>(), c->d_plan_sums.as<unsigned long long>(), s.d_wa + 8, sa, c->hp_briefs);
    c->sig_seq++;
    launch_plan(s.d_briefs, n, s.d_distinct, c->d_slot_rank.as<uint32_t>(), c->slot_mask, c->d_plan_sums.as<unsigned long long>(), c->d_plans.as<ChangePlan>(),
                c->d_plans.as<ChangePlan>() + s.n1, s.d_wa, s.d_wa + 8, s.sig, c->sig_seq, sa, s.spec_possible ? c->d_plan_totals.as<PlanTotals>() : nullptr,
                c->h_s1.as<uint32_t>());
    const bool want_large_spec = s.spec_possible && attempt == 0 && c->hint_large != 0;
    if (want_large_spec) HIPCHK(c, hipEventRecord(c->ev_plan, sa));
    if (s.spec_possible && attempt == 0) {
      const uint64_t est = c->raw.size() / 2 + 1024;
      c->spec_cap_ops = (uint32_t)std::min<uint64_t>(std::max<uint64_t>(c->hint_ops, est), 0x7ffffff0u);
      c->spec_cap_preds = (uint32_t)std::min<uint64_t>(std::max<uint64_t>(c->hint_preds, est), 0x7ffffff0u);
      if (lap.on) fprintf(stderr, "replay: speculative decode: cap %u ops / %u preds (counter block %zu of %zu bytes)\n", c->spec_cap_ops, c->spec_cap_preds, merge_counts_bytes(c->spec_cap_ops), s.counts_bytes);
      if (merge_counts_bytes(c->spec_cap_ops) <= s.counts_bytes && carve_cols(c, c->spec_cap_ops, c->spec_cap_preds, true) == AM355_OK) {
        canary_arm();
        if (c->phase_events) { HIPCHK(c, hipEventRecord(c->ev[1], sa)); HIPCHK(c, hipEventRecord(c->ev[2], sa)); }
        if (want_large_spec) HIPCHK(c, hipStreamWaitEvent(c->stream3, c->ev_plan, 0));
        launch_decode_speculative(c->d_arena.as<uint8_t>(), c->d_metas.as<ChangeMeta>(), c->d_plans.as<ChangePlan>(), n, c->d_plan_totals.as<PlanTotals>(), c->spec_cap_ops,
                                  c->spec_cap_preds, distinct_capacity(), c->d_amap_prov.as<uint32_t>(), c->d_slot_rank.as<uint32_t>(), c->cols,
                                  &c->d_counts.as<Counts>()->flags, sa, c->stream3, want_large_spec, c->shard_rank, c->shard_world);
        c->spec_large_launched = want_large_spec;
        if (c->phase_events) HIPCHK(c, hipEventRecord(c->ev[3], sa));
        c->spec_launched = true;
      }
    }
    if (c->phase_events && !c->spec_launched) HIPCHK(c, hipEventRecord(c->ev[1], sa));
    if (attempt == 0 && !s.hash_enqueued) { int rb = replay_enqueue_hash_stream(c, s); if (rb) return rb; s.hash_enqueued = true; }
    lap("stage 1 enqueued");
    if (!wait_host_signal(&s.sig->plan_seq, c->sig_seq, sa)) {
      (void)hipStreamSynchronize(c->stream2);
      (void)hipStreamSynchronize(c->stream3);
      return fail(c, AM355_E_DEVICE, "the device did not report the plan of this replay (%s)", hipGetErrorString(hipGetLastError()));
    }
    memcpy(&s.tot, (const void*)&s.sig->plan, sizeof s.tot);
    lap("stage 1 totals read");
    if (!(s.tot.fast_a & FF_CAPACITY) || attempt) break;
    c->spec_launched = false;
    c->amap_cap = s.tot.total_entries + 1024;
    if (!c->d_amap_prov.ensure(4 * (size_t)c->amap_cap)) return fail(c, AM355_E_NOMEM, "device allocation failed (actor tables)");
    HIPCHK(c, hipMemsetAsync(s.d_wa + W_FAST_A, 0, 4, sa));
    HIPCHK(c, hipMemsetAsync(s.d_wa + 8, 0, 32, sa));
  }
  return AM355_OK;
}

static int replay_stage1_verdict(am355_ctx* c, Stage1& s) {
  const PlanTotals& tot = s.tot;
  s.t_host0 = std::chrono::steady_clock::now();
  if (tot.flags_a) { (void)hipStreamSynchronize(c->stream); (void)hipStreamSynchronize(c->stream2); return error_for_flags(c, tot.flags_a, "malformed change"); }
  c->has_unknown_cols = tot.reserved[0] != 0;
  s.fast = tot.fast_a == 0;
  s.lineage_schedule = c->in_apply && c->graph_mode != 0;
  if (s.lineage_schedule) s.fast = false;
  if (tot.n_distinct > distinct_capacity()) s.fast = false;
  s.planned = !tot.fallback && !getenv("AM355_HOST_PLAN");
  if (tot.fallback) {
    const ChangeBrief* br = c->hp_briefs;
    uint32_t dev_flags = 0;
    c->has_unknown_cols = false;
    for (uint32_t i = 0; i < s.n; i++) {
      dev_flags |= br[i].flags_fits & 0x1fffffffu;
      if (br[i].flags_fits & 0x20000000u) c->has_unknown_cols = true;
    }
    if (dev_flags) { (void)hipStreamSynchronize(c->stream); (void)hipStreamSynchronize(c->stream2); return error_for_flags(c, dev_flags, "malformed change"); }
  }
  return AM355_OK;
}

static void replay_optimistic(am355_ctx* c, Stage1& s, const TraceLap& lap) {
  if (!s.fast) return;
  if (s.planned) {
    float ms_plan = 0;
    s.opt_rc = run_device_planned(c, s.tot, s.tot.n_distinct, &ms_plan);
    s.ms_host += ms_plan;
    lap("run_device (device plan) done");
  } else {
    std::vector<uint32_t> slot_rank;
    s.opt_rc = plan_fast(c, slot_rank);
    s.ms_host += std::chrono::duration<float, std::milli>(std::chrono::steady_clock::now() - s.t_host0).count();
    lap("plan_fast done");
    if (s.opt_rc == AM355_OK) s.opt_rc = run_device(c, &slot_rank);
    lap("run_device done");
  }
  s.opt_flags = c->flags;
  s.opt_err = c->err;
}

static int replay_join_hash_stream(am355_ctx* c, Stage1& s, const TraceLap& lap) {
  if (s.lane_join.l) { s.lane_join.l->wait(); s.lane_join.l = nullptr; if (s.lane_rc.load()) return s.lane_rc.load(); }
// ... 170 lines not shown
```

### automerge_classic_amd/engine.py

```python
import ctypes
import os

import numpy as np

_HERE = os.path.dirname(os.path.abspath(__file__))
DEFAULT_LIB = os.path.join(_HERE, "csrc", "libam355.so")

AM355_OK = 0
AM355_E_DEVICE, AM355_E_ARG, AM355_E_INVALID, AM355_E_UNSUPPORTED, AM355_E_STATE, AM355_E_NOMEM = -1, -2, -3, -4, -5, -6

FLAG_NAMES = {
    1 << 0: "BAD_MAGIC", 1 << 1: "BAD_CHECKSUM", 1 << 2: "BAD_CHUNK", 1 << 3: "BAD_COLUMNS", 1 << 4: "BAD_LEB", 1 << 5: "BAD_RLE",
    1 << 6: "BAD_ROW", 1 << 7: "UNKNOWN_OBJECT", 1 << 8: "BAD_ELEM", 1 << 9: "BAD_PRED", 1 << 10: "DUP_OPID", 1 << 11: "BAD_COUNTER",
    1 << 12: "UNSUPPORTED", 1 << 13: "OVERFLOW", 1 << 16: "BAD_SEQ", 1 << 17: "UNKNOWN_ACTOR", 1 << 18: "BAD_DEFLATE",
}


class Stats(ctypes.Structure):
    _fields_ = [
        ("n_changes", ctypes.c_uint32), ("n_applied", ctypes.c_uint32), ("n_pending", ctypes.c_uint32),
        ("n_actors", ctypes.c_uint32), ("n_objects", ctypes.c_uint32), ("n_heads", ctypes.c_uint32),
        ("n_ops", ctypes.c_uint64), ("max_op", ctypes.c_uint64), ("raw_bytes", ctypes.c_uint64),
        ("n_map_values", ctypes.c_uint64), ("n_list_elems", ctypes.c_uint64), ("n_edits", ctypes.c_uint64),
        ("ir_bytes", ctypes.c_uint64),
# ... 211 lines not shown
        deps = np.frombuffer(b"".join(bytes.fromhex(h) for h in request["deps"]), dtype=np.uint8).copy()
        if deps.size != 32 * len(request["deps"]):
            raise _NotFlat("deps")
        for f in ("seq", "startOp", "time"):
            if not isinstance(request[f], int) or isinstance(request[f], bool) or abs(request[f]) >= 2 ** 63:
                raise _NotFlat(f)
        if request["seq"] < 0 or request["startOp"] < 0:
            raise _NotFlat("seq / startOp")
    except (_NotFlat, KeyError, TypeError, ValueError, AttributeError, UnicodeEncodeError):
        lc.not_flat = 1
        return lc, keep
    lc.seq, lc.start_op, lc.time = request["seq"], request["startOp"], request["time"]
    msg = np.frombuffer(message, dtype=np.uint8).copy()
    lc.message, lc.message_len = arr(msg), msg.size
    lc.deps, lc.n_deps = arr(deps), deps.size // 32
    offs = np.zeros(len(table) + 1, dtype=np.uint32)
    np.cumsum([len(a) for a in table], out=offs[1:])
    lc.n_actors = len(table)
    lc.actor_off = arr(offs)
    lc.actor_bytes = arr(np.frombuffer(b"".join(table), dtype=np.uint8).copy())
    lc.actor_rank = arr(rank)
    st = np.frombuffer(bytes(strings), dtype=np.uint8).copy()
    lc.strings, lc.strings_len = arr(st), st.size
    ops = np.ascontiguousarray(ops)
    lc.ops, lc.n_ops = arr(ops), ops.shape[0]
    lc.values, lc.n_values = arr(val_arr), val_arr.size
    lc.preds, lc.n_preds = arr(pred_arr), pred_arr.shape[0]
    return lc, keep


def _bind(path):
    if not os.path.exists(path):
        raise RuntimeError(f"HIP engine library not found: {path}. Build it with `python -c 'import __graft_entry__ as g; g.build()'` "
                           "(hipcc --offload-arch=gfx950). There is no CPU fallback.")
    L = ctypes.CDLL(path)
    vp, u32, u64p = ctypes.c_void_p, ctypes.c_uint32, ctypes.c_void_p
    L.am355_create.restype = vp
    L.am355_create.argtypes = [ctypes.c_int]
    L.am355_destroy.argtypes = [vp]
    L.am355_last_error.restype = ctypes.c_char_p
    L.am355_last_error.argtypes = [vp]
    L.am355_flags.restype = u32
    L.am355_flags.argtypes = [vp]
    L.am355_load_changes.argtypes = [vp, vp, u64p, u32]
    L.am355_load_document.argtypes = [vp, vp, ctypes.c_size_t]
    if hasattr(L, "am355_backend_load"):
        L.am355_backend_load.argtypes = [vp, vp, ctypes.c_size_t]
        L.am355_backend_load.restype = ctypes.c_int
    L.am355_replay.argtypes = [vp]
    L.am355_patch_json.argtypes = [vp, ctypes.POINTER(ctypes.c_char_p), ctypes.POINTER(ctypes.c_size_t)]
    L.am355_get_stats.argtypes = [vp, ctypes.POINTER(Stats)]
    L.am355_get_hashes.argtypes = [vp, vp]
    L.am355_test_sort.argtypes = [vp, vp, vp, u32, ctypes.c_int]
    L.am355_test_scan.argtypes = [vp, vp, vp, u32, vp]
    sz, ci = ctypes.c_size_t, ctypes.c_int
    for f, args in (("am355_test_scan_at", [vp, vp, u32, u32, vp, u32, u32, u32, vp]), ("am355_test_scan2", [vp, vp, vp, u32, u32, vp, vp, u32, u32, u32, vp, vp]),
                    ("am355_test_scan_terminators", [vp, vp, sz, u32, u32, vp, u32, u32, vp]), ("am355_test_max", [vp, vp, u32, vp]),
                    ("am355_test_sort_bits", [vp, vp, vp, u32, ci, ci, vp, ctypes.POINTER(ci)]), ("am355_test_chain_mark", [vp, vp, vp, u32, u32]),
                    ("am355_test_remap", [vp, vp, u32, u32, vp, u32, vp, u32, ctypes.POINTER(u32)]), ("am355_test_fill", [vp, vp, u32, u32, vp, u32, ctypes.POINTER(u32)]),
                    ("am355_test_copy", [vp, vp, sz, vp, sz, ci, vp, u32, ctypes.POINTER(u32)]), ("am355_test_signal_words", [vp, vp, u32, vp, u32, u32, vp, u32, vp]),
                    ("am355_test_carried_scan", [vp, vp, u32, vp, vp, vp]), ("am355_test_text_premises", [vp, vp, u32, u32, u32, u32, ctypes.POINTER(u32), ctypes.POINTER(u32)])):
        if not hasattr(L, f):
            continue
        getattr(L, f).argtypes = args
        getattr(L, f).restype = ci
    L.am355_get_rows.argtypes = [vp] * 15
    L.am355_save.argtypes = [vp, u32, ctypes.POINTER(ctypes.c_void_p), ctypes.POINTER(ctypes.c_size_t)]
    L.am355_get_applied.argtypes = [vp, vp, ctypes.POINTER(u32)]
    L.am355_fetch_ir.argtypes = [vp, vp]
    L.am355_set_shard.argtypes = [vp, u32, u32]
    L.am355_fragment_size.argtypes = [vp, ctypes.POINTER(ctypes.c_size_t)]
    L.am355_export_fragment.argtypes = [vp, vp, ctypes.c_size_t, ctypes.c_int, ctypes.POINTER(ctypes.c_size_t)]
    L.am355_import_fragments.argtypes = [vp, vp, vp, u32]
    L.am355_shard_unique_id.argtypes = [vp]
    L.am355_shard_init.argtypes = [vp, vp, u32, u32]
    L.am355_sharded_replay.argtypes = [vp, ctypes.c_int]
    L.am355_shard_fragment_bytes.argtypes = [vp, vp, u32]
    L.am355_shard_finalize.argtypes = [vp]
    for f in ("am355_shard_unique_id", "am355_shard_init", "am355_sharded_replay", "am355_shard_fragment_bytes", "am355_shard_finalize"):
        getattr(L, f).restype = ctypes.c_int
    if hasattr(L, "am355_resident_counters"):
        L.am355_resident_counters.argtypes = [vp, vp]
        L.am355_resident_counters.restype = ctypes.c_int
    if hasattr(L, "am355_resident_maps_only_calls"):
        L.am355_resident_maps_only_calls.argtypes = [vp, ctypes.POINTER(ctypes.c_uint64)]
        L.am355_resident_maps_only_calls.restype = ctypes.c_int
    if hasattr(L, "am355_set_resident_new_actors"):
        L.am355_set_resident_new_actors.argtypes = [vp, ctypes.c_int]
        L.am355_set_resident_new_actors.restype = ctypes.c_int
        L.am355_resident_new_actor_calls.argtypes = [vp, vp]
        L.am355_resident_new_actor_calls.restype = ctypes.c_int
    if hasattr(L, "am355_set_resident_new_objects"):
        L.am355_set_resident_new_objects.argtypes = [vp, ctypes.c_int]
        L.am355_set_resident_new_objects.restype = ctypes.c_int
        L.am355_resident_new_object_calls.argtypes = [vp, vp]
        L.am355_resident_new_object_calls.restype = ctypes.c_int
    if hasattr(L, "am355_set_resident_counters"):
        L.am355_set_resident_counters.argtypes = [vp, ctypes.c_int]
        L.am355_set_resident_counters.restype = ctypes.c_int
        L.am355_resident_counter_calls.argtypes = [vp, vp]
        L.am355_resident_counter_calls.restype = ctypes.c_int
    if hasattr(L, "am355_set_resident_map_merge"):
        L.am355_set_resident_map_merge.argtypes = [vp, ctypes.c_int]
        L.am355_set_resident_map_merge.restype = ctypes.c_int
        L.am355_resident_map_merge_calls.argtypes = [vp, vp]
        L.am355_resident_map_merge_calls.restype = ctypes.c_int
    if hasattr(L, "am355_apply_local_change"):
        L.am355_encode_change.argtypes = [vp, ctypes.POINTER(LocalChange), ctypes.POINTER(ctypes.c_void_p), ctypes.POINTER(ctypes.c_size_t), vp]
        L.am355_apply_local_change.argtypes = [vp, ctypes.POINTER(LocalChange), ctypes.POINTER(ctypes.c_void_p), ctypes.POINTER(ctypes.c_size_t)]
        L.am355_local_change_calls.argtypes = [vp, vp]
        for f in ("am355_encode_change", "am355_apply_local_change", "am355_local_change_calls"):
            getattr(L, f).restype = ctypes.c_int
    if hasattr(L, "am355_set_local_small"):
        L.am355_set_local_small.argtypes = [vp, ctypes.c_int]
        L.am355_set_local_small.restype = ctypes.c_int
        L.am355_local_small_calls.argtypes = [vp, vp]
        L.am355_local_small_calls.restype = ctypes.c_int
    if hasattr(L, "am355_changes_added"):
        L.am355_find_changes.argtypes = [vp, vp, u32, vp]
        for f in ("am355_changes_since", "am355_changes_added", "am355_missing_deps"):
            getattr(L, f).argtypes = [vp, vp, u32, ctypes.POINTER(ctypes.c_void_p), ctypes.POINTER(u32)]
        L.am355_set_graph_probe_min.argtypes = [vp, u32]
        L.am355_graph_query_calls.argtypes = [vp, vp]
        L.am355_test_hash_probe.argtypes = [vp, vp, u32, vp, u32, vp]
        for f in ("am355_find_changes", "am355_changes_since", "am355_changes_added", "am355_missing_deps", "am355_set_graph_probe_min", "am355_graph_query_calls",
                  "am355_test_hash_probe"):
            getattr(L, f).restype = ctypes.c_int
    if hasattr(L, "am355_object_text"):
        L.am355_object_text.argtypes = [vp, ctypes.c_uint64, vp, ctypes.c_size_t, ctypes.POINTER(ctypes.c_void_p), ctypes.POINTER(ctypes.c_size_t), ctypes.POINTER(TextInfo)]
        L.am355_object_text_calls.argtypes = [vp, vp]
        L.am355_set_text_pinned_max.argtypes = [vp, ctypes.c_uint64]
        L.am355_text_limits.argtypes = [vp]
        for f in ("am355_object_text", "am355_object_text_calls", "am355_set_text_pinned_max", "am355_text_limits"):
            getattr(L, f).restype = ctypes.c_int
    if hasattr(L, "am355_text_splice"):
        L.am355_text_locate.argtypes = [vp, ctypes.c_uint64, vp, ctypes.c_size_t, ctypes.c_uint64, ctypes.c_uint64, ctypes.POINTER(ctypes.c_void_p), ctypes.POINTER(u32),
                                        ctypes.POINTER(ctypes.c_uint64)]
        L.am355_text_splice.argtypes = [vp, ctypes.c_uint64, vp, ctypes.c_size_t, ctypes.c_uint64, ctypes.c_uint64, vp, vp, u32, vp, ctypes.c_size_t, ctypes.c_int64, vp, u32,
                                        ctypes.POINTER(ctypes.c_void_p), ctypes.POINTER(ctypes.c_size_t)]
        L.am355_text_splice_calls.argtypes = [vp, vp]
        L.am355_text_locate_limits.argtypes = [vp]
        for f in ("am355_text_locate", "am355_text_splice", "am355_text_splice_calls", "am355_text_locate_limits"):
            getattr(L, f).restype = ctypes.c_int
    if hasattr(L, "am355_list_splice"):
        pvp, psz = ctypes.POINTER(ctypes.c_void_p), ctypes.POINTER(ctypes.c_size_t)
        L.am355_list_locate.argtypes = [vp, ctypes.c_uint64, vp, ctypes.c_size_t, ctypes.c_uint64, ctypes.c_uint64, pvp, ctypes.POINTER(u32), pvp, ctypes.POINTER(u32),
                                        ctypes.POINTER(ctypes.c_uint64)]
        L.am355_list_splice.argtypes = [vp, ctypes.c_uint64, vp, ctypes.c_size_t, ctypes.c_uint64, ctypes.c_uint64, vp, u32, vp, u32, vp, ctypes.c_size_t, ctypes.c_int64, vp, u32,
                                        pvp, psz]
        L.am355_list_set.argtypes = [vp, ctypes.c_uint64, vp, ctypes.c_size_t, ctypes.c_uint64, vp, vp, u32, vp, ctypes.c_size_t, ctypes.c_int64, vp, u32, pvp, psz]
        L.am355_list_splice_calls.argtypes = [vp, vp]
        L.am355_list_locate_limits.argtypes = [vp]
        L.am355_test_list_premises.argtypes = [vp, vp, u32, u32, u32, u32, ctypes.POINTER(u32), ctypes.POINTER(u32)]
        for f in ("am355_list_locate", "am355_list_splice", "am355_list_set", "am355_list_splice_calls", "am355_list_locate_limits", "am355_test_list_premises"):
            getattr(L, f).restype = ctypes.c_int
    if hasattr(L, "am355_text_position"):
        L.am355_text_position.argtypes = [vp, ctypes.c_uint64, vp, ctypes.c_size_t, vp, u32, ctypes.POINTER(ctypes.c_void_p), ctypes.POINTER(ctypes.c_uint64)]
        L.am355_rank_of_actor.argtypes = [vp, vp, ctypes.c_size_t, ctypes.POINTER(u32)]
        L.am355_actor_of_rank.argtypes = [vp, u32, ctypes.POINTER(ctypes.c_void_p), ctypes.POINTER(ctypes.c_size_t)]
        L.am355_actor_of_rank.restype = ctypes.c_int
        L.am355_text_position_calls.argtypes = [vp, vp]
        L.am355_text_position_limits.argtypes = [vp]
        for f in ("am355_text_position", "am355_rank_of_actor", "am355_text_position_calls", "am355_text_position_limits"):
            getattr(L, f).restype = ctypes.c_int
    L.am355_get_raw.argtypes = [vp, ctypes.POINTER(ctypes.c_void_p), ctypes.POINTER(ctypes.c_void_p), ctypes.POINTER(u32)]
    L.am355_doc_changes.argtypes = [vp, u32, ctypes.POINTER(ctypes.c_void_p), ctypes.POINTER(ctypes.c_void_p), ctypes.POINTER(u32), ctypes.POINTER(ctypes.c_void_p)]
# ... 383 lines not shown
        t, q = self._hash_rows(table_hashes), self._hash_rows(queries)
        out = np.full(q.shape[0], 0x55555555, dtype=np.uint32)
        self._check(self._L.am355_test_hash_probe(self._h, t.ctypes.data if t.size else None, t.shape[0], q.ctypes.data if q.size else None, q.shape[0],
                                                  out.ctypes.data if q.size else None))
        return out

    def apply_patch_json(self):
        p = ctypes.c_char_p()
        n = ctypes.c_size_t()
        self._check(self._L.am355_apply_patch_json(self._h, ctypes.byref(p), ctypes.byref(n)))
        return ctypes.string_at(p, n.value).decode("utf-8")

    def fetch_ir(self):
        self._check(self._L.am355_fetch_ir(self._h, None))

    def patch_json(self):
        p = ctypes.c_char_p()
        n = ctypes.c_size_t()
        self._check(self._L.am355_patch_json(self._h, ctypes.byref(p), ctypes.byref(n)))
        return ctypes.string_at(p, n.value).decode("utf-8")

    def save(self, reencode=False):
        p = ctypes.c_void_p()
        n = ctypes.c_size_t()
        self._check(self._L.am355_save(self._h, 1 if reencode else 0, ctypes.byref(p), ctypes.byref(n)))
        return ctypes.string_at(p, n.value)

    def applied(self):
        n = ctypes.c_uint32()
        self._check(self._L.am355_get_applied(self._h, None, ctypes.byref(n)))
        out = np.zeros(n.value, dtype=np.uint32)
        self._check(self._L.am355_get_applied(self._h, out.ctypes.data if n.value else None, ctypes.byref(n)))
        return out

    def stats(self):
        s = Stats()
        self._check(self._L.am355_get_stats(self._h, ctypes.byref(s)))
        return s

    def set_shard(self, rank, world):
        self._check(self._L.am355_set_shard(self._h, rank, world))

    def fragment_size(self):
        n = ctypes.c_size_t()
        self._check(self._L.am355_fragment_size(self._h, ctypes.byref(n)))
        return n.value

    def export_fragment(self, ptr, capacity, device):
        n = ctypes.c_size_t()
        self._check(self._L.am355_export_fragment(self._h, ctypes.c_void_p(ptr), capacity, 1 if device else 0, ctypes.byref(n)))
        return n.value

    def import_fragments(self, frags, offsets):
        f = np.ascontiguousarray(frags, dtype=np.uint8)
        o = np.ascontiguousarray(offsets, dtype=np.uint64)
        self._check(self._L.am355_import_fragments(self._h, f.ctypes.data, o.ctypes.data, o.size - 1))

    def shard_unique_id(self):
        buf = (ctypes.c_uint8 * 128)()
        if self._L.am355_shard_unique_id(buf) != AM355_OK:
            raise EngineError(AM355_E_DEVICE, "RCCL is not available (librccl.so.1, or AM355_RCCL_LIB)")
        return bytes(buf)

    def shard_init(self, unique_id, rank, world):
        assert len(unique_id) == 128
        self._check(self._L.am355_shard_init(self._h, ctypes.c_char_p(bytes(unique_id)), rank, world))

    def sharded_replay(self, stitch_on_all_ranks=False):
        self._check(self._L.am355_sharded_replay(self._h, 1 if stitch_on_all_ranks else 0))

    def shard_fragment_bytes(self, world):
        out = np.zeros(world, dtype=np.uint64)
        self._check(self._L.am355_shard_fragment_bytes(self._h, out.ctypes.data, world))
        return out

    def shard_finalize(self):
        self._check(self._L.am355_shard_finalize(self._h))

    def resident_counters(self):
        out = (ctypes.c_uint64 * 3)()
        self._check(self._L.am355_resident_counters(self._h, out))
        return int(out[0]), int(out[1]), int(out[2])

    def resident_maps_only_calls(self):
        out = ctypes.c_uint64()
        self._check(self._L.am355_resident_maps_only_calls(self._h, ctypes.byref(out)))
        return int(out.value)

    def set_resident_new_actors(self, on):
        self._check(self._L.am355_set_resident_new_actors(self._h, 1 if on else 0))

    def resident_new_actor_calls(self):
        out = (ctypes.c_uint64 * 2)()
        self._check(self._L.am355_resident_new_actor_calls(self._h, out))
        return int(out[0]), int(out[1])

    def set_resident_map_merge(self, on):
        self._check(self._L.am355_set_resident_map_merge(self._h, 1 if on else 0))

    def resident_map_merge_calls(self):
        out = (ctypes.c_uint64 * 2)()
        self._check(self._L.am355_resident_map_merge_calls(self._h, out))
        return int(out[0]), int(out[1])

    def set_resident_new_objects(self, on):
        self._check(self._L.am355_set_resident_new_objects(self._h, 1 if on else 0))

    def resident_new_object_calls(self):
        out = (ctypes.c_uint64 * 2)()
        self._check(self._L.am355_resident_new_object_calls(self._h, out))
        return int(out[0]), int(out[1])

    def set_resident_counters(self, on):
        self._check(self._L.am355_set_resident_counters(self._h, 1 if on else 0))

    def resident_counter_calls(self):
        out = (ctypes.c_uint64 * 2)()
        self._check(self._L.am355_resident_counter_calls(self._h, out))
        return int(out[0]), int(out[1])

    def raw(self):
        a, o, n = ctypes.c_void_p(), ctypes.c_void_p(), ctypes.c_uint32()
        self._check(self._L.am355_get_raw(self._h, ctypes.byref(a), ctypes.byref(o), ctypes.byref(n)))
        offs = np.ctypeslib.as_array(ctypes.cast(o, ctypes.POINTER(ctypes.c_uint64)), shape=(n.value + 1,)).copy()
        size = int(offs[-1])
        arena = np.ctypeslib.as_array(ctypes.cast(a, ctypes.POINTER(ctypes.c_uint8)), shape=(size,)).copy() if size else np.zeros(0, dtype=np.uint8)
        return arena, offs

    def doc_changes(self, deflate=True):
        a, o, n, h = ctypes.c_void_p(), ctypes.c_void_p(), ctypes.c_uint32(), ctypes.c_void_p()
        self._check(self._L.am355_doc_changes(self._h, 1 if deflate else 0, ctypes.byref(a), ctypes.byref(o), ctypes.byref(n), ctypes.byref(h)))
        offs = np.ctypeslib.as_array(ctypes.cast(o, ctypes.POINTER(ctypes.c_uint64)), shape=(n.value + 1,)).copy()
        size = int(offs[-1])
        arena = np.ctypeslib.as_array(ctypes.cast(a, ctypes.POINTER(ctypes.c_uint8)), shape=(size,)).copy() if size else np.zeros(0, dtype=np.uint8)
        hashes = np.ctypeslib.as_array(ctypes.cast(h, ctypes.POINTER(ctypes.c_uint8)), shape=(n.value, 32)).copy() if n.value else np.zeros((0, 32), dtype=np.uint8)
        return arena, offs, hashes

    def hashes(self):
        out = np.zeros((self._n_changes, 32), dtype=np.uint8)
        self._check(self._L.am355_get_hashes(self._h, out.ctypes.data))
        return out

    def test_sort(self, keys, vals, key_bits=64):
        k = np.ascontiguousarray(keys, dtype=np.uint64).copy()
        v = np.ascontiguousarray(vals, dtype=np.uint32).copy()
        self._check(self._L.am355_test_sort(self._h, k.ctypes.data, v.ctypes.data, k.size, key_bits))
        return k, v

    def test_scan(self, values):
        a = np.ascontiguousarray(values, dtype=np.uint32)
        out = np.zeros_like(a)
        total = np.zeros(1, dtype=np.uint32)
        self._check(self._L.am355_test_scan(self._h, a.ctypes.data, out.ctypes.data, a.size, total.ctypes.data))
        return out, int(total[0])

    @staticmethod
    def _img(a, dtype=np.uint32):
        return None if a is None else np.ascontiguousarray(a, dtype=dtype).copy()

    @staticmethod
    def _ptr(a):
        return None if a is None else a.ctypes.data

    def prim_scan(self, in_buf, in_off, n, out_buf=None, out_off=0, total=None):
        a, o = self._img(in_buf), self._img(out_buf)
        t = None if total is None else np.array([total], dtype=np.uint32)
# ... 97 lines not shown
```

### include/am355.h

```cpp
#ifndef AM355_H
#define AM355_H
#include <stddef.h>
#include <stdint.h>

#ifdef __cplusplus
extern "C" {
#endif

typedef struct am355_ctx am355_ctx;

enum {
  AM355_OK = 0,
  AM355_E_DEVICE = -1,
  AM355_E_ARG = -2,
  AM355_E_INVALID = -3,
  AM355_E_UNSUPPORTED = -4,
  AM355_E_STATE = -5,
  AM355_E_NOMEM = -6
};

enum {
  AM355_F_BAD_MAGIC = 1u << 0, AM355_F_BAD_CHECKSUM = 1u << 1, AM355_F_BAD_CHUNK = 1u << 2, AM355_F_BAD_COLUMNS = 1u << 3,
  AM355_F_BAD_LEB = 1u << 4, AM355_F_BAD_RLE = 1u << 5, AM355_F_BAD_ROW = 1u << 6, AM355_F_UNKNOWN_OBJECT = 1u << 7,
  AM355_F_BAD_ELEM = 1u << 8, AM355_F_BAD_PRED = 1u << 9, AM355_F_DUP_OPID = 1u << 10, AM355_F_BAD_COUNTER = 1u << 11,
// ... 93 lines not shown
  const uint8_t *arena;
  uint64_t arena_len;
} am355_patch_ir;
int am355_fetch_ir(am355_ctx *ctx, am355_patch_ir *out);

int am355_apply_changes(am355_ctx *ctx, const uint8_t *arena, const uint64_t *offsets, uint32_t n_changes);
int am355_reset(am355_ctx *ctx);
int am355_forget_call_history(am355_ctx *ctx, int from_document);
int am355_hash_graph_known(am355_ctx *ctx, int set, int *known);

int am355_get_pending(const am355_ctx *ctx, uint32_t *out, uint32_t *n_pending);
int am355_apply_patch_json(am355_ctx *ctx, const char **json, size_t *len);
int am355_fetch_apply_ir(am355_ctx *ctx, am355_patch_ir *out);

enum { AM355_LK_STRING = 0, AM355_LK_HEAD = 1, AM355_LK_ELEM = 2 };
enum { AM355_LOP_INSERT = 1u, AM355_LOP_VALUES = 2u };
enum { AM355_LV_NULL = 0, AM355_LV_FALSE = 1, AM355_LV_TRUE = 2, AM355_LV_UINT = 3, AM355_LV_INT = 4, AM355_LV_FLOAT64 = 5,
       AM355_LV_UTF8 = 6, AM355_LV_BYTES = 7, AM355_LV_COUNTER = 8, AM355_LV_TIMESTAMP = 9,
       AM355_LV_BAD = 15  };
typedef struct {
  uint32_t action;
  uint32_t obj_actor, obj_ctr;
  uint32_t key_kind;
  uint32_t key_off, key_len;
  uint32_t elem_actor, elem_ctr;
  uint32_t flags;
  uint32_t multi;
  uint32_t val_first;
  uint32_t pred_first, pred_num;
} am355_local_op;
typedef struct {
  uint32_t tag;
  uint32_t off, len;
  uint32_t pad;
  uint64_t payload;
} am355_local_value;
typedef struct { uint32_t actor, ctr; } am355_local_pred;
typedef struct {
  uint64_t seq, start_op;
  int64_t time;
  const uint8_t *message; uint32_t message_len;
  const uint8_t *deps; uint32_t n_deps;
  uint32_t n_actors;
  const uint32_t *actor_off;
  const uint8_t *actor_bytes;
  const uint32_t *actor_rank;
  const uint8_t *strings; uint32_t strings_len;
  const am355_local_op *ops; uint32_t n_ops;
  const am355_local_value *values; uint32_t n_values;
  const am355_local_pred *preds; uint32_t n_preds;
  uint32_t not_flat;
} am355_local_change;
int am355_encode_change(am355_ctx *ctx, const am355_local_change *request, const uint8_t **bytes, size_t *len, uint8_t hash[32]);
int am355_apply_local_change(am355_ctx *ctx, const am355_local_change *request, const uint8_t **change, size_t *len);
int am355_local_change_calls(const am355_ctx *ctx, uint64_t out[2]);
int am355_set_local_small(am355_ctx *ctx, int on);
int am355_local_small_calls(const am355_ctx *ctx, uint64_t out[2]);
typedef struct {
  uint32_t is_local;
  uint32_t actor;
  uint64_t seq;
} am355_local_envelope;
int am355_apply_local_envelope(const am355_ctx *ctx, am355_local_envelope *out);

int am355_get_dep_graph(am355_ctx *ctx, const uint32_t **dep_first, const uint32_t **dep_index, uint32_t *n_changes);
int am355_sync_bloom_build(am355_ctx *ctx, const uint32_t *idx, uint32_t n, uint8_t *bits, size_t capacity);
int am355_sync_bloom_probe(am355_ctx *ctx, const uint32_t *idx, uint32_t n, uint32_t num_entries, uint32_t bits_per_entry, uint32_t num_probes,
                           const uint8_t *bits, size_t n_bytes, uint8_t *contains);

int am355_set_shard(am355_ctx *ctx, uint32_t rank, uint32_t world);
int am355_fragment_size(am355_ctx *ctx, size_t *bytes);
int am355_export_fragment(am355_ctx *ctx, void *dst, size_t capacity, int dst_is_device, size_t *len);
int am355_import_fragments(am355_ctx *ctx, const uint8_t *frags, const uint64_t *offsets, uint32_t world);

#define AM355_SHARD_ID_BYTES 128
int am355_shard_unique_id(uint8_t id[AM355_SHARD_ID_BYTES]);
int am355_shard_init(am355_ctx *ctx, const uint8_t id[AM355_SHARD_ID_BYTES], uint32_t rank, uint32_t world);
int am355_sharded_replay(am355_ctx *ctx, int stitch_on_all_ranks);
int am355_shard_fragment_bytes(am355_ctx *ctx, uint64_t *bytes, uint32_t capacity);
int am355_shard_finalize(am355_ctx *ctx);

int am355_resident_counters(const am355_ctx *ctx, uint64_t out[3]);
int am355_resident_maps_only_calls(const am355_ctx *ctx, uint64_t *out);
int am355_set_resident_new_actors(am355_ctx *ctx, int on);
int am355_resident_new_actor_calls(const am355_ctx *ctx, uint64_t out[2]);
int am355_set_resident_map_merge(am355_ctx *ctx, int on);
int am355_resident_map_merge_calls(const am355_ctx *ctx, uint64_t out[2]);
int am355_set_resident_new_objects(am355_ctx *ctx, int on);
int am355_resident_new_object_calls(const am355_ctx *ctx, uint64_t out[2]);
int am355_set_resident_counters(am355_ctx *ctx, int on);
int am355_resident_counter_calls(const am355_ctx *ctx, uint64_t out[2]);

int am355_arena_epoch(const am355_ctx *ctx, uint64_t *epoch);
int am355_get_hashes_range(const am355_ctx *ctx, uint32_t first, uint32_t count, uint8_t *out);
int am355_applied_in_input_order(const am355_ctx *ctx, int *yes);

int am355_find_changes(am355_ctx *ctx, const uint8_t *hashes, uint32_t n, uint32_t *out_idx);
int am355_changes_since(am355_ctx *ctx, const uint8_t *have, uint32_t n_have, const uint32_t **idx, uint32_t *n);
int am355_changes_added(am355_ctx *ctx, const uint8_t *other, uint32_t n_other, const uint32_t **idx, uint32_t *n);
int am355_missing_deps(am355_ctx *ctx, const uint8_t *heads, uint32_t n_heads, const uint8_t **hashes, uint32_t *n);
int am355_set_graph_probe_min(am355_ctx *ctx, uint32_t n);
int am355_graph_query_calls(const am355_ctx *ctx, uint64_t out[2]);

typedef struct { uint32_t n_elements, n_strings; uint64_t bytes; } am355_text_info;
int am355_object_text(am355_ctx *ctx, uint64_t obj_ctr, const uint8_t *obj_actor, size_t actor_len,
                      const uint8_t **utf8, size_t *len, am355_text_info *info );
int am355_object_text_calls(const am355_ctx *ctx, uint64_t out[2]);
int am355_set_text_pinned_max(am355_ctx *ctx, uint64_t bytes);
int am355_text_limits(uint32_t out[4]);

enum { AM355_RUN_COUNTER = 1u };
typedef struct { uint32_t elem_ctr, elem_actor, pred_ctr, pred_actor, count, flags; } am355_text_run;
int am355_text_locate(am355_ctx *ctx, uint64_t obj_ctr, const uint8_t *obj_actor, size_t actor_len,
                      uint64_t first, uint64_t n, const am355_text_run **runs, uint32_t *n_runs, uint64_t *length);
int am355_text_splice(am355_ctx *ctx, uint64_t obj_ctr, const uint8_t *obj_actor, size_t actor_len,
                      uint64_t start, uint64_t deletions,
                      const uint8_t *utf8, const uint32_t *value_off, uint32_t n_values,
                      const uint8_t *author, size_t author_len, int64_t time, const uint8_t *message, uint32_t message_len,
                      const uint8_t **change, size_t *len);
int am355_text_splice_calls(const am355_ctx *ctx, uint64_t out[3]);
int am355_text_locate_limits(uint32_t out[3]);
int am355_actor_of_rank(const am355_ctx *ctx, uint32_t rank, const uint8_t **bytes, size_t *len);

typedef struct { uint32_t elem_ctr, elem_actor, count, flags, pred_first, pred_num; } am355_list_run;
typedef struct { uint32_t actor, ctr; } am355_list_pred;
int am355_list_locate(am355_ctx *ctx, uint64_t obj_ctr, const uint8_t *obj_actor, size_t actor_len, uint64_t first, uint64_t n,
                      const am355_list_run **runs, uint32_t *n_runs, const am355_list_pred **preds, uint32_t *n_preds, uint64_t *length);
int am355_list_splice(am355_ctx *ctx, uint64_t obj_ctr, const uint8_t *obj_actor, size_t actor_len, uint64_t start, uint64_t deletions,
                      const am355_local_value *values, uint32_t n_values, const uint8_t *strings, uint32_t strings_len,
                      const uint8_t *author, size_t author_len, int64_t time, const uint8_t *message, uint32_t message_len,
                      const uint8_t **change, size_t *len);
int am355_list_set(am355_ctx *ctx, uint64_t obj_ctr, const uint8_t *obj_actor, size_t actor_len, uint64_t index,
                   const am355_local_value *value, const uint8_t *strings, uint32_t strings_len,
                   const uint8_t *author, size_t author_len, int64_t time, const uint8_t *message, uint32_t message_len,
                   const uint8_t **change, size_t *len);
int am355_list_splice_calls(const am355_ctx *ctx, uint64_t out[3]);
int am355_list_locate_limits(uint32_t out[3]);

enum { AM355_POS_UNKNOWN = 0u, AM355_POS_VISIBLE = 1u, AM355_POS_DELETED = 2u, AM355_POS_STATUS = 3u , AM355_POS_COUNTER = 0x100u };
typedef struct { uint32_t ctr, actor; } am355_elem_id;
typedef struct { uint32_t position, status; } am355_elem_pos;
int am355_text_position(am355_ctx *ctx, uint64_t obj_ctr, const uint8_t *obj_actor, size_t actor_len,
                        const am355_elem_id *ids, uint32_t n, const am355_elem_pos **out, uint64_t *length);
int am355_rank_of_actor(const am355_ctx *ctx, const uint8_t *bytes, size_t len, uint32_t *rank);
int am355_text_position_calls(const am355_ctx *ctx, uint64_t out[2]);
int am355_text_position_limits(uint32_t out[2]);

int am355_test_hash_probe(am355_ctx *ctx, const uint8_t *table_hashes, uint32_t n_table, const uint8_t *queries, uint32_t n_queries, uint32_t *out_idx);
int am355_test_sort(am355_ctx *ctx, uint64_t *keys, uint32_t *vals, uint32_t n, int key_bits);
int am355_test_scan(am355_ctx *ctx, const uint32_t *in, uint32_t *out, uint32_t n, uint32_t *total);
int am355_test_scan_at(am355_ctx *ctx, uint32_t *in_buf, uint32_t in_words, uint32_t in_off, uint32_t *out_buf, uint32_t out_words, uint32_t out_off,
                       uint32_t n, uint32_t *total);
int am355_test_scan2(am355_ctx *ctx, uint32_t *in_a, uint32_t *in_b, uint32_t in_words, uint32_t in_off, uint32_t *out_a, uint32_t *out_b, uint32_t out_words,
                     uint32_t out_off, uint32_t n, uint32_t *total_a, uint32_t *total_b);
int am355_test_scan_terminators(am355_ctx *ctx, const uint8_t *bytes_buf, size_t bytes_len, uint32_t byte_off, uint32_t L, uint32_t *out_buf, uint32_t out_words,
                                uint32_t out_off, uint32_t *total);
int am355_test_max(am355_ctx *ctx, const uint32_t *v, uint32_t n, uint32_t *inout);
int am355_test_sort_bits(am355_ctx *ctx, uint64_t *keys, uint32_t *vals, uint32_t n, int begin_bit, int end_bit, const uint32_t *first_table, int *result_buffer);
int am355_test_chain_mark(am355_ctx *ctx, const uint32_t *next, uint32_t *mark, uint32_t mark_words, uint32_t n);
int am355_test_remap(am355_ctx *ctx, uint32_t *buf, uint32_t words, uint32_t base_off, const uint32_t *ranges, uint32_t n_ranges, const uint32_t *table, uint32_t n_old,
                     uint32_t *n_added);
int am355_test_fill(am355_ctx *ctx, uint32_t *buf, uint32_t words, uint32_t base_off, const uint32_t *ranges, uint32_t n_ranges, uint32_t *n_added);
int am355_test_copy(am355_ctx *ctx, uint8_t *dst, size_t dst_bytes, const uint8_t *src, size_t src_bytes, int src_pinned, const uint32_t *ranges, uint32_t n_ranges,
                    uint32_t *n_added);
int am355_test_signal_words(am355_ctx *ctx, const uint32_t *a, uint32_t n_a, const uint32_t *b, uint32_t n_b, uint32_t seq, uint32_t *host_words, uint32_t host_words_n,
                            uint32_t *seq_word);
// ... 12 lines not shown
```

Measured before the change: 1.231 billion.

## Build actor spans and offset table on device during planning to skip host upload

Per-author change counts are now gathered with wave-aggregated atomics in the actor check kernel. The plan kernel scans those counts into an actor table offset array and scatters each change's ActorSpan by sequence number on the device. When the host confirms changes arrived in sequence order, merge resolve is enqueued right after the fills and the host span staging and upload are skipped. If the host ordering disagrees, decode and fills are rerun, which adds cost on that path along with extra shared memory and atomics in the plan kernels.

```diff
diff --git a/automerge_classic_amd/csrc/am355_api.hip b/automerge_classic_amd/csrc/am355_api.hip
--- a/automerge_classic_amd/csrc/am355_api.hip
+++ b/automerge_classic_amd/csrc/am355_api.hip
@@ -115,6 +115,31 @@
   return AM355_OK;
 }
 
+extern "C" int am355_device_span_counters(const am355_ctx* c, uint64_t out[3]) {
+  if (!c || !out) return AM355_E_ARG;
+  out[0] = c->n_dev_spans;
+  out[1] = c->n_host_spans;
+  out[2] = c->n_dev_spans_redone;
+  return AM355_OK;
+}
+
+extern "C" int am355_test_spans(am355_ctx* c, uint32_t* dev_spans, uint32_t* host_spans, uint32_t cap_spans, uint32_t* dev_tab, uint32_t* host_tab, uint32_t cap_tab,
+                                uint32_t* n_spans, uint32_t* n_tab) {
+  if (!c || !n_spans || !n_tab) return AM355_E_ARG;
+  if (!c->replayed || c->is_document || !c->p_spans || !c->p_tab_off) return AM355_E_STATE;
+  const size_t ns = c->spans.size(), nt = c->actor_tab_off.size();
+  *n_spans = (uint32_t)ns;
+  *n_tab = (uint32_t)nt;
+  if (ns > cap_spans || nt > cap_tab) return AM355_E_ARG;
+  (void)hipSetDevice(c->device);
+  HIPCHK(c, hipStreamSynchronize(c->stream));
+  if (host_spans && ns) memcpy(host_spans, c->spans.data(), sizeof(ActorSpan) * ns);
+  if (host_tab && nt) memcpy(host_tab, c->actor_tab_off.data(), 4 * nt);
+  if (dev_spans && ns) HIPCHK(c, hipMemcpy(dev_spans, c->p_spans, sizeof(ActorSpan) * ns, hipMemcpyDeviceToHost));
+  if (dev_tab && nt) HIPCHK(c, hipMemcpy(dev_tab, c->p_tab_off, 4 * nt, hipMemcpyDeviceToHost));
+  return AM355_OK;
+}
+
 extern "C" int am355_resident_maps_only_calls(const am355_ctx* c, uint64_t* out) {
   if (!c || !out) return AM355_E_ARG;
   *out = c->n_maps_only_calls;
diff --git a/automerge_classic_amd/csrc/am355_ctx.h b/automerge_classic_amd/csrc/am355_ctx.h
--- a/automerge_classic_amd/csrc/am355_ctx.h
+++ b/automerge_classic_amd/csrc/am355_ctx.h
@@ -416,6 +416,10 @@
   DevBuf d_plans, d_amap, d_tables;
   ActorSpan* p_spans = nullptr;
   uint32_t* p_tab_off = nullptr;
+  DevBuf d_span_cnt;
+  void* dev_spans_at = nullptr;
+  bool spans_by_seq = false;
+  uint64_t n_dev_spans = 0, n_host_spans = 0, n_dev_spans_redone = 0;
 
   DevBuf d_cols, d_pred, d_merge, d_sort, d_ir, d_counts;
   OpCols cols{};
diff --git a/automerge_classic_amd/csrc/am355_decode.h b/automerge_classic_amd/csrc/am355_decode.h
--- a/automerge_classic_amd/csrc/am355_decode.h
+++ b/automerge_classic_amd/csrc/am355_decode.h
@@ -2,10 +2,11 @@
 #include "am355_internal.h"
 
 namespace am355 {
+constexpr uint32_t PARSE_FILLS_MAX = 8;
 struct ParseFills {
-  uint32_t* p[5];
-  uint64_t n_words[5];
-  uint32_t value[5];
+  uint32_t* p[PARSE_FILLS_MAX];
+  uint64_t n_words[PARSE_FILLS_MAX];
+  uint32_t value[PARSE_FILLS_MAX];
   uint32_t n;
 };
 void parse_changes_host(const uint8_t* arena, const uint64_t* offsets, uint32_t n_changes, ChangeMeta* metas, uint32_t* n_entries);
@@ -19,13 +20,15 @@
 void launch_actor_intern(const uint8_t* arena, ChangeMeta* metas, uint32_t n, const uint32_t* amap_base, uint32_t* amap, uint32_t amap_cap,
                          unsigned long long* slots, uint32_t slot_mask, uint32_t* first_idx, uint32_t* flags, uint32_t* fast_flags, uint32_t* distinct,
                          void* rank_ids, ChangeBrief* briefs, uint32_t* slot_rank, unsigned long long* block_sums, uint32_t* plan_words, hipStream_t st,
-                         ChangeBrief* host_briefs = nullptr);
+                         ChangeBrief* host_briefs = nullptr, uint32_t* span_cnt = nullptr);
 size_t rank_ids_bytes();
 size_t plan_block_sums_bytes(uint32_t n);
 uint32_t distinct_capacity();
 void launch_plan(const ChangeBrief* briefs, uint32_t n, const uint32_t* distinct, const uint32_t* slot_rank, uint32_t slot_mask, const unsigned long long* block_sums,
                  ChangePlan* plans, ChangePlan* plans_serial, const uint32_t* words, const uint32_t* plan_words, HostSignals* sig, uint32_t seq, hipStream_t st,
-                 PlanTotals* dev_totals = nullptr, uint32_t* host_s1 = nullptr);
+                 PlanTotals* dev_totals = nullptr, uint32_t* host_s1 = nullptr, const uint32_t* span_cnt = nullptr, ActorSpan* spans = nullptr,
+                 uint32_t* tab_off = nullptr);
+uint32_t plan_rank_max();
 void launch_decode_speculative(const uint8_t* arena, const ChangeMeta* metas, const ChangePlan* plans, uint32_t n_changes, const PlanTotals* totals, uint32_t cap_ops,
                                uint32_t cap_preds, uint32_t cap_distinct, const uint32_t* amap, const uint32_t* slot_rank, OpCols cols, uint32_t* flags, hipStream_t st,
                                hipStream_t aux, bool with_large, uint32_t shard_rank = 0, uint32_t shard_world = 1);
diff --git a/automerge_classic_amd/csrc/am355_decode.hip b/automerge_classic_amd/csrc/am355_decode.hip
--- a/automerge_classic_amd/csrc/am355_decode.hip
+++ b/automerge_classic_amd/csrc/am355_decode.hip
@@ -1093,7 +1093,7 @@
                                                        const uint32_t* __restrict__ first_idx, uint32_t* __restrict__ flags, uint32_t* __restrict__ fast_flags,
                                                        ChangeBrief* __restrict__ briefs, const uint32_t* __restrict__ distinct, const RankId* __restrict__ rank_ids,
                                                        uint32_t* __restrict__ slot_rank, unsigned long long* __restrict__ block_sums, uint32_t* __restrict__ plan_words,
-                                                       ChangeBrief* __restrict__ host_briefs) {
+                                                       ChangeBrief* __restrict__ host_briefs, uint32_t* __restrict__ span_cnt, uint32_t slot_mask) {
   wave_priority_high();
   __shared__ unsigned long long s_scan[BLOCK / WAVE][3];
   if (blockIdx.x + 1 == gridDim.x) {
@@ -1134,10 +1134,23 @@
     bad |= ob;
     unknown |= ou;
   }
+  const unsigned long long m_empty = __ballot(valid && !has);
+  if (span_cnt) {
+    const bool counted = valid && br.author_slot <= slot_mask;
+    const unsigned long long m = __ballot(counted);
+    if (m) {
+      const uint32_t leader = (uint32_t)__ffsll(m) - 1;
+      const uint32_t s0 = __shfl(br.author_slot, (int)leader);
+      const bool one_author = __ballot(counted && br.author_slot != s0) == 0;
+      if (one_author) { if ((threadIdx.x & (WAVE - 1)) == leader) atomicAdd(&span_cnt[s0], (uint32_t)__popcll(m)); }
+      else if (counted) atomicAdd(&span_cnt[br.author_slot], 1u);
+    }
+  }
   if ((threadIdx.x & (WAVE - 1)) == 0) {
     if (mx_op) atomicMax(&plan_words[1], mx_op);
     if (bad) atomicOr(&plan_words[2], bad);
     if (unknown) atomicOr(&plan_words[3], 1u);
+    if (m_empty) atomicOr(&plan_words[4], 1u);
   }
   if (threadIdx.x == 0) {
     unsigned long long* out = block_sums + (size_t)blockIdx.x * PLAN_SUMS;
@@ -1149,10 +1162,21 @@
                                                       const unsigned long long* __restrict__ block_sums, ChangePlan* __restrict__ plans,
                                                       ChangePlan* __restrict__ plans_serial, const uint32_t* __restrict__ words, const uint32_t* __restrict__ plan_words,
                                                       const uint32_t* __restrict__ distinct, HostSignals* sig, uint32_t seq, PlanTotals* __restrict__ dev_totals,
-                                                      uint32_t* __restrict__ host_s1) {
+                                                      uint32_t* __restrict__ host_s1, const uint32_t* __restrict__ span_cnt, ActorSpan* __restrict__ spans,
+                                                      uint32_t* __restrict__ tab_off) {
   wave_priority_high();
   __shared__ unsigned long long s_scan[BLOCK / WAVE][3];
   __shared__ unsigned long long s_base[6];
+  constexpr uint32_t SPAN_PER = PLAN_RANK_MAX / BLOCK;
+  __shared__ uint32_t s_tab[PLAN_RANK_MAX + 1];
+  __shared__ uint32_t s_wave_sum[BLOCK / WAVE];
+  uint32_t span_slot[SPAN_PER], nd = 0;
+  if (spans) {
+#pragma unroll
+    for (uint32_t k = 0; k < SPAN_PER; k++) span_slot[k] = distinct[1 + threadIdx.x + k * BLOCK];
+    nd = distinct[0];
+  }
+  const bool build_spans = spans && nd <= PLAN_RANK_MAX && !plan_words[0] && !plan_words[4];
   {
     unsigned long long p0 = 0, p1 = 0, p2 = 0, p3 = 0, p4 = 0, p5 = 0;
     for (uint32_t j = threadIdx.x; j < blockIdx.x; j += BLOCK) {
@@ -1175,12 +1199,49 @@
   unsigned long long e1[3], e2[3], t1[3], t2[3];
   block_scan3(valid ? br.n_ops : 0u, valid ? br.n_preds : 0u, valid ? br.n_entries : 0u, s_scan, e1, t1);
   block_scan3(small ? 1u : 0u, large ? 1u : 0u, serial ? 1u : 0u, s_scan, e2, t2);
+  const bool slot_ok = has && br.author_slot <= slot_mask;
+  const uint32_t author_rank = slot_ok ? slot_rank[br.author_slot] : 0u, op_base = (uint32_t)(s_base[0] + e1[0]);
   if (has) {
-    ChangePlan pl{c, (uint32_t)(s_base[0] + e1[0]), (uint32_t)(s_base[1] + e1[1]), (uint32_t)(s_base[2] + e1[2]),
-                  br.author_slot <= slot_mask ? slot_rank[br.author_slot] : 0u, br.n_entries};
+    ChangePlan pl{c, op_base, (uint32_t)(s_base[1] + e1[1]), (uint32_t)(s_base[2] + e1[2]), author_rank, br.n_entries};
     if (small) plans[(uint32_t)(s_base[3] + e2[0])] = pl;
     else if (large) plans[n - 1 - (uint32_t)(s_base[4] + e2[1])] = pl;
     else plans_serial[(uint32_t)(s_base[5] + e2[2])] = pl;
+  }
+  if (build_spans) {
+    const uint32_t t = threadIdx.x, lane = t & (WAVE - 1), w = t / WAVE;
+    for (uint32_t i = t; i <= PLAN_RANK_MAX; i += BLOCK) s_tab[i] = 0;
+    __syncthreads();
+#pragma unroll
+    for (uint32_t k = 0; k < SPAN_PER; k++) {
+      const uint32_t a = t + k * BLOCK, slot = span_slot[k];
+      if (a < nd && slot <= slot_mask) {
+        const uint32_t r = slot_rank[slot];
+        if (r < nd) s_tab[r] = span_cnt[slot];
+      }
+    }
+    __syncthreads();
+    uint32_t v[SPAN_PER], sum = 0;
+#pragma unroll
+    for (uint32_t k = 0; k < SPAN_PER; k++) { v[k] = s_tab[SPAN_PER * t + k]; sum += v[k]; }
+    uint32_t incl = sum;
+    for (int d = 1; d < WAVE; d <<= 1) {
+      const uint32_t y = __shfl_up(incl, (unsigned)d);
+      if (lane >= (uint32_t)d) incl += y;
+    }
+    if (lane == WAVE - 1) s_wave_sum[w] = incl;
+    __syncthreads();
+    uint32_t run = incl - sum;
+    for (uint32_t k = 0; k < w; k++) run += s_wave_sum[k];
+#pragma unroll
+    for (uint32_t k = 0; k < SPAN_PER; k++) { s_tab[SPAN_PER * t + k] = run; run += v[k]; }
+    if (t == BLOCK - 1) s_tab[PLAN_RANK_MAX] = run;
+    __syncthreads();
+    if (blockIdx.x == 0)
+      for (uint32_t i = t; i <= nd; i += BLOCK) tab_off[i] = s_tab[i];
+    if (slot_ok && author_rank < nd) {
+      const uint32_t first = s_tab[author_rank], cnt = s_tab[author_rank + 1] - first;
+      if (br.seq >= 1 && br.seq <= cnt) spans[first + (uint32_t)br.seq - 1] = ActorSpan{br.start_op, br.n_ops, op_base};
+    }
   }
   if (blockIdx.x + 1 == gridDim.x && host_s1) {
     const uint32_t nd = distinct[0] < DISTINCT_CAP ? distinct[0] : DISTINCT_CAP;
@@ -1203,6 +1264,7 @@
     z.fallback = (plan_words[0] || ops >= 0x7ffffff0ull || preds >= 0xfffffff0ull || ent >= 0xfffffff0ull) ? 1u : 0u;
     z.flags_a = words[0] | plan_words[2]; z.fast_a = words[1]; z.total_entries = words[2]; z.n_distinct = distinct[0];
     z.reserved[0] = plan_words[3];
+    z.reserved[1] = build_spans && !z.fallback ? 1u : 0u;
     if (dev_totals) *dev_totals = z;
     signal_host((uint32_t*)&sig->plan, (const uint32_t*)&z, sizeof(PlanTotals) / 4, &sig->plan_seq, seq);
   }
@@ -2222,14 +2284,14 @@
 void launch_actor_intern(const uint8_t* arena, ChangeMeta* metas, uint32_t n, const uint32_t* amap_base, uint32_t* amap, uint32_t amap_cap,
                          unsigned long long* slots, uint32_t slot_mask, uint32_t* first_idx, uint32_t* flags, uint32_t* fast_flags, uint32_t* distinct,
                          void* rank_ids, ChangeBrief* briefs, uint32_t* slot_rank, unsigned long long* block_sums, uint32_t* plan_words, hipStream_t st,
-                         ChangeBrief* host_briefs) {
+                         ChangeBrief* host_briefs, uint32_t* span_cnt) {
   if (n)
     hipLaunchKernelGGL(k_actor_intern, dim3(n), dim3(WAVE), 0, st, arena, metas, n, amap_base, amap, amap_cap, slots, slot_mask, first_idx, flags,
                        fast_flags, distinct, (RankId*)rank_ids);
   if (n) hipLaunchKernelGGL(k_actor_first, dim3(n), dim3(WAVE), 0, st, metas, n, amap_base, (const uint32_t*)amap, amap_cap, (const uint32_t*)first_idx, fast_flags);
   hipLaunchKernelGGL(k_actor_check, dim3((n + BLOCK - 1) / BLOCK + 1), dim3(BLOCK), 0, st, arena, metas, n, amap_base, (const uint32_t*)amap, amap_cap,
                      (const uint32_t*)first_idx, flags, fast_flags, briefs, (const uint32_t*)distinct, (const RankId*)rank_ids, slot_rank, block_sums, plan_words,
-                     host_briefs);
+                     host_briefs, span_cnt, slot_mask);
 }
 
 size_t rank_ids_bytes() { return sizeof(RankId) * PLAN_RANK_MAX; }
@@ -2238,13 +2300,15 @@
 
 void launch_plan(const ChangeBrief* briefs, uint32_t n, const uint32_t* distinct, const uint32_t* slot_rank, uint32_t slot_mask, const unsigned long long* block_sums,
                  ChangePlan* plans, ChangePlan* plans_serial, const uint32_t* words, const uint32_t* plan_words, HostSignals* sig, uint32_t seq, hipStream_t st,
-                 PlanTotals* dev_totals, uint32_t* host_s1) {
+                 PlanTotals* dev_totals, uint32_t* host_s1, const uint32_t* span_cnt, ActorSpan* spans, uint32_t* tab_off) {
+  if (!span_cnt || !tab_off) spans = nullptr;
   uint32_t nb = (n + BLOCK - 1) / BLOCK;
   hipLaunchKernelGGL(k_plan_apply, dim3(nb ? nb : 1), dim3(BLOCK), 0, st, briefs, n, slot_rank, slot_mask, block_sums, plans, plans_serial, words, plan_words,
-                     distinct, sig, seq, dev_totals, host_s1);
+                     distinct, sig, seq, dev_totals, host_s1, span_cnt, spans, tab_off);
 }
 
 uint32_t distinct_capacity() { return DISTINCT_CAP; }
+uint32_t plan_rank_max() { return PLAN_RANK_MAX; }
 
 __global__ __launch_bounds__(WAVE) void k_doc_count(const uint8_t* __restrict__ arena, ChangeMeta* __restrict__ meta) {
   uint32_t lane = threadIdx.x;
diff --git a/automerge_classic_amd/csrc/am355_replay.hip b/automerge_classic_amd/csrc/am355_replay.hip
--- a/automerge_classic_amd/csrc/am355_replay.hip
+++ b/automerge_classic_amd/csrc/am355_replay.hip
@@ -23,6 +23,7 @@
     size_t k_n = c->actor_tab_off[a + 1] - c->actor_tab_off[a];
     bool sorted = true;
     for (size_t k = 1; k < k_n; k++) sorted = sorted && v[k - 1].start_op <= v[k].start_op;
+    if (!sorted) c->spans_by_seq = false;
     if (!sorted) std::sort(v, v + k_n, [](const ActorSpan& x, const ActorSpan& y) { return x.start_op < y.start_op; });
     for (size_t k = 1; k < k_n; k++)
       if ((uint64_t)v[k - 1].start_op + v[k - 1].n_ops > v[k].start_op) {
@@ -384,6 +385,7 @@
   c->applied_change.resize(n);
   c->applied_op_base.resize(n);
   c->pass_first_row.clear();
+  c->spans_by_seq = order == nullptr;
   uint64_t ops = 0, preds = 0, entries = 0, max_op = 0;
   for (uint32_t t = 0; t < n; t++) {
     const uint32_t ci = order ? order[t] : t;
@@ -399,7 +401,7 @@
       c->plans.push_back(ChangePlan{ci, (uint32_t)ops, (uint32_t)preds, (uint32_t)entries, author, m.n_entries});
       span_cnt[author]++;
       max_op = std::max<uint64_t>(max_op, (uint64_t)m.start_op + m.n_ops - 1);
-    }
+    } else c->spans_by_seq = false;
     ops += m.n_ops;
     preds += m.n_preds;
     entries += m.n_entries;
@@ -523,9 +525,9 @@
 
 static void take_counts(am355_ctx* c, const Counts* hc) { c->counts = *hc; c->counts.n_objects += 1; }
 
-static int merge_and_take_counts(am355_ctx* c) {
+static int merge_and_take_counts(am355_ctx* c, bool resolved = false) {
   Counts* hc = c->h_counts.as<Counts>();
-  merge_run(c->mb, c->ir, hc, c->stream, (c->phase_events || !c->mb.sig) ? c->ev_counts.h : nullptr, c->ev_runs);
+  merge_run(c->mb, c->ir, hc, c->stream, (c->phase_events || !c->mb.sig) ? c->ev_counts.h : nullptr, c->ev_runs, resolved);
   HIPCHK(c, hipEventRecord(c->ev[5], c->stream));
   if (hc->flags) return error_for_flags(c, hc->flags, "op set rejected");
   take_counts(c, hc);
@@ -555,6 +557,7 @@
   c->sig_seq++;
   int rcb = setup_buffers(c, (uint32_t)c->actors.size());
   if (rcb) return rcb;
+  if (c->n_ops) c->n_host_spans++;
   uint32_t n_small = 0, n_large = 0;
   {
     const ChangeBrief* br = c->hp_briefs;
@@ -603,6 +606,8 @@
 }
 
 struct GeneralOrder { const uint32_t* order; const uint32_t* pass; uint32_t n_applied; hipEvent_t ready; };
+static size_t planned_tab_offset(uint32_t n) { return (sizeof(ActorSpan) * (size_t)n + 16 + 255) & ~(size_t)255; }
+static size_t planned_tables_bytes(uint32_t n, uint32_t n_distinct) { return planned_tab_offset(n) + ((4 * ((size_t)n_distinct + 1) + 16 + 255) & ~(size_t)255); }
 static int run_device_planned(am355_ctx* c, const PlanTotals& tot, uint32_t n_distinct, float* ms_host_plan, const GeneralOrder* go = nullptr) {
   hipStream_t st = c->stream;
   const TraceLap lap("  planned:", 26);
@@ -611,12 +616,13 @@
   c->n_ops = tot.n_ops;
   c->n_preds = tot.n_preds;
   c->max_op = tot.max_op;
-  auto al = [](size_t b) { return (b + 255) & ~(size_t)255; };
-  size_t o_tab = al(sizeof(ActorSpan) * (size_t)n + 16), tables_bytes = o_tab + al(4 * ((size_t)n_distinct + 1) + 16);
+  const size_t o_tab = planned_tab_offset(n), tables_bytes = planned_tables_bytes(n, n_distinct);
   if (!c->d_tables.ensure(tables_bytes) || !c->h_stage.ensure(tables_bytes)) return fail(c, AM355_E_NOMEM, "device allocation failed");
   uint8_t* d_tables = c->d_tables.as<uint8_t>();
   c->p_spans = (ActorSpan*)d_tables;
   c->p_tab_off = (uint32_t*)(d_tables + o_tab);
+  const bool dev_spans = !go && c->shard_world <= 1 && tot.reserved[1] && tot.n_ops && n_distinct <= plan_rank_max() && c->dev_spans_at && c->dev_spans_at == c->d_tables.p;
+  c->dev_spans_at = nullptr;
   c->sig_seq++;
   int rcb = setup_buffers(c, n_distinct);
   if (rcb) return rcb;
@@ -636,6 +642,28 @@
   if (!spec_done && !(c->counts_zeroed_at == c->d_counts.p && c->mb.counts_bytes <= c->counts_zeroed)) HIPCHK(c, hipMemsetAsync(c->d_counts.p, 0, c->mb.counts_bytes, st));
   c->counts_zeroed_at = nullptr;
   c->hint_large = tot.n_large;
+  auto decode_ordinary = [&]() -> int {
+    if (tot.n_small && (tot.n_large || tot.n_serial)) {
+      HIPCHK(c, hipEventRecord(c->ev_fork, st));
+      HIPCHK(c, hipStreamWaitEvent(c->stream3, c->ev_fork, 0));
+    }
+    if (c->phase_events) HIPCHK(c, hipEventRecord(c->ev[2], st));
+    launch_decode_planned(c->d_arena.as<uint8_t>(), c->d_metas.as<ChangeMeta>(), c->d_plans.as<ChangePlan>(), c->d_plans.as<ChangePlan>() + std::max(n, 1u), n,
+                          tot.n_small, tot.n_large, tot.n_serial, c->d_amap_prov.as<uint32_t>(), c->d_slot_rank.as<uint32_t>(), c->cols,
+                          &c->d_counts.as<Counts>()->flags, st, c->stream3, c->shard_rank, c->shard_world);
+    if (c->phase_events) HIPCHK(c, hipEventRecord(c->ev[3], st));
+    return AM355_OK;
+  };
+  const bool second_class = tot.n_small && (tot.n_large || tot.n_serial);
+  hipStream_t fill_stream = second_class ? c->stream4 : c->stream3;
+  auto fills_and_join = [&]() -> int {
+    if (!merge_prepare(c->mb, fill_stream)) return fail(c, AM355_E_DEVICE, "merge fills: more ranges than one launch takes");
+    if (second_class) {
+      HIPCHK(c, hipEventRecord(c->ev_join, c->stream3));
+      HIPCHK(c, hipStreamWaitEvent(st, c->ev_join, 0));
+    }
+    return AM355_OK;
+  };
   if (spec_done) {
     c->hint_ops = std::max(c->hint_ops, tot.n_ops);
     c->hint_preds = std::max(c->hint_preds, tot.n_preds);
@@ -653,26 +681,20 @@
   } else {
     c->hint_ops = tot.n_ops;
     c->hint_preds = tot.n_preds;
-    if (tot.n_small && (tot.n_large || tot.n_serial)) {
-      HIPCHK(c, hipEventRecord(c->ev_fork, st));
-      HIPCHK(c, hipStreamWaitEvent(c->stream3, c->ev_fork, 0));
-    }
-    if (c->phase_events) HIPCHK(c, hipEventRecord(c->ev[2], st));
-    launch_decode_planned(c->d_arena.as<uint8_t>(), c->d_metas.as<ChangeMeta>(), c->d_plans.as<ChangePlan>(), c->d_plans.as<ChangePlan>() + std::max(n, 1u), n,
-                          tot.n_small, tot.n_large, tot.n_serial, c->d_amap_prov.as<uint32_t>(), c->d_slot_rank.as<uint32_t>(), c->cols,
-                          &c->d_counts.as<Counts>()->flags, st, c->stream3, c->shard_rank, c->shard_world);
+    int rcd = decode_ordinary();
+    if (rcd) return rcd;
     lap("decode launched");
-    if (c->phase_events) HIPCHK(c, hipEventRecord(c->ev[3], st));
   }
   c->spec_launched = false;
-  const bool second_class = tot.n_small && (tot.n_large || tot.n_serial);
-  hipStream_t fill_stream = second_class ? c->stream4 : c->stream3;
-  if (!merge_prepare(c->mb, fill_stream)) return fail(c, AM355_E_DEVICE, "merge fills: more ranges than one launch takes");
-  if (second_class) {
-    HIPCHK(c, hipEventRecord(c->ev_join, c->stream3));
-    HIPCHK(c, hipStreamWaitEvent(st, c->ev_join, 0));
-  }
+  int rcf = fills_and_join();
+  if (rcf) return rcf;
   lap("fills enqueued");
+  if (dev_spans) {
+    HIPCHK(c, hipEventRecord(c->ev_tables, fill_stream));
+    HIPCHK(c, hipStreamWaitEvent(st, c->ev_tables, 0));
+    merge_resolve(c->mb, st);
+    lap("k_resolve enqueued");
+  }
   if (go) HIPCHK(c, hipEventSynchronize(go->ready));
   auto t0 = std::chrono::steady_clock::now();
   std::vector<uint32_t> slot_rank;
@@ -682,6 +704,17 @@
   if (rc == AM355_OK && (c->n_ops != tot.n_ops || c->n_preds != tot.n_preds || c->max_op != tot.max_op || c->actors.size() != n_distinct))
     rc = fail(c, AM355_E_DEVICE, "internal: device and host plans disagree (%llu / %u ops)", (unsigned long long)c->n_ops, tot.n_ops);
   if (rc) { (void)hipStreamSynchronize(st); return rc; }
+  if (dev_spans && c->spans_by_seq) {
+    c->n_dev_spans++;
+    return merge_and_take_counts(c, true);
+  }
+  if (dev_spans) {
+    c->n_dev_spans_redone++;
+    HIPCHK(c, hipStreamSynchronize(st));
+    HIPCHK(c, hipMemsetAsync(c->d_counts.p, 0, c->mb.counts_bytes, st));
+    if ((rc = decode_ordinary()) || (rc = fills_and_join())) return rc;
+    lap("decode and fills enqueued again");
+  } else if (tot.n_ops) c->n_host_spans++;
   {
     uint8_t* h = c->h_stage.as<uint8_t>();
     size_t b_spans = sizeof(ActorSpan) * c->spans.size(), b_tab = 4 * c->actor_tab_off.size();
@@ -1740,6 +1773,13 @@
       !c->d_slot_rank.ensure(4 * (size_t)(c->slot_mask + 1)) || !c->d_plan_sums.ensure(plan_block_sums_bytes(n)) ||
       !c->d_dep_idx.ensure(4 * (c->raw.size() / 32 + 2)) || !c->d_self_idx.ensure(4 * n1) || !c->d_rank_ids.ensure(rank_ids_bytes()))
     return fail(c, AM355_E_NOMEM, "device allocation failed (stage 1)");
+  c->dev_spans_at = nullptr;
+  if (n && c->shard_world <= 1 && !getenv("AM355_HOST_PLAN") && !(c->in_apply && c->graph_mode != 0)) {
+    if (!c->d_span_cnt.ensure(4 * (size_t)(c->slot_mask + 1)) || !c->d_tables.ensure(planned_tables_bytes(n, distinct_capacity())))
+      return fail(c, AM355_E_NOMEM, "device allocation failed (stage 1)");
+    c->dev_spans_at = c->d_tables.p;
+    c->resident_valid = false;
+  }
   c->have_host_metas = false;
   const size_t s1_briefs = S1_DISTINCT + ((12 * (size_t)distinct_capacity() + 16 + 63) & ~(size_t)63);
   const size_t s1_bytes = s1_briefs + sizeof(ChangeBrief) * n1;
@@ -1769,6 +1809,11 @@
   add(c->d_slots.p, 8 * (size_t)(c->slot_mask + 1), 0);
   add(c->d_first_idx.p, 4 * (size_t)(c->slot_mask + 1), 0xffffffffu);
   if (s.counts_cleared) add(c->d_counts.p, s.counts_bytes, 0);
+  if (c->dev_spans_at) {
+    add(c->d_span_cnt.p, 4 * (size_t)(c->slot_mask + 1), 0);
+    add(c->dev_spans_at, sizeof(ActorSpan) * (size_t)s.n, 0);
+  }
+  static_assert(PARSE_FILLS_MAX >= 7, "replay_parse: fill ranges");
   launch_parse_changes(c->d_arena.as<uint8_t>(), c->d_offsets.as<uint64_t>(), s.n, c->d_metas.as<ChangeMeta>(), c->d_entries.as<uint32_t>(), f, sa, s.fat_changes);
   HIPCHK(c, hipEventRecord(c->ev_parse, sa));
   if (s.counts_cleared) {
@@ -1811,17 +1856,20 @@
   s.spec_possible = n && s.counts_cleared && !getenv("AM355_HOST_PLAN") && !(c->in_apply && c->graph_mode != 0) && c->d_plan_totals.ensure(sizeof(PlanTotals));
   for (int attempt = 0;; attempt++) {
     if (attempt) {
+      c->dev_spans_at = nullptr;
       HIPCHK(c, hipMemsetAsync(c->d_slots.p, 0, 8 * (size_t)(c->slot_mask + 1), sa));
       HIPCHK(c, hipMemsetAsync(c->d_first_idx.p, 0xff, 4 * (size_t)(c->slot_mask + 1), sa));
       HIPCHK(c, hipMemsetAsync(s.d_distinct, 0, 4, sa));
     }
     launch_actor_intern(c->d_arena.as<uint8_t>(), c->d_metas.as<ChangeMeta>(), n, c->d_amap_base.as<uint32_t>(), c->d_amap_prov.as<uint32_t>(), c->amap_cap,
                         c->d_slots.as<unsigned long long>(), c->slot_mask, c->d_first_idx.as<uint32_t>(), s.d_wa + W_FLAGS_A, s.d_wa + W_FAST_A,
-                        s.d_distinct, c->d_rank_ids.p, s.d_briefs, c->d_slot_rank.as<uint32_t>(), c->d_plan_sums.as<unsigned long long>(), s.d_wa + 8, sa, c->hp_briefs);
+                        s.d_distinct, c->d_rank_ids.p, s.d_briefs, c->d_slot_rank.as<uint32_t>(), c->d_plan_sums.as<unsigned long long>(), s.d_wa + 8, sa, c->hp_briefs,
+                        c->dev_spans_at ? c->d_span_cnt.as<uint32_t>() : nullptr);
     c->sig_seq++;
     launch_plan(s.d_briefs, n, s.d_distinct, c->d_slot_rank.as<uint32_t>(), c->slot_mask, c->d_plan_sums.as<unsigned long long>(), c->d_plans.as<ChangePlan>(),
                 c->d_plans.as<ChangePlan>() + s.n1, s.d_wa, s.d_wa + 8, s.sig, c->sig_seq, sa, s.spec_possible ? c->d_plan_totals.as<PlanTotals>() : nullptr,
-                c->h_s1.as<uint32_t>());
+                c->h_s1.as<uint32_t>(), c->dev_spans_at ? c->d_span_cnt.as<uint32_t>() : nullptr, (ActorSpan*)c->dev_spans_at,
+                c->dev_spans_at ? (uint32_t*)((uint8_t*)c->dev_spans_at + planned_tab_offset(n)) : nullptr);
     const bool want_large_spec = s.spec_possible && attempt == 0 && c->hint_large != 0;
     if (want_large_spec) HIPCHK(c, hipEventRecord(c->ev_plan, sa));
     if (s.spec_possible && attempt == 0) {
diff --git a/automerge_classic_amd/engine.py b/automerge_classic_amd/engine.py
--- a/automerge_classic_amd/engine.py
+++ b/automerge_classic_amd/engine.py
@@ -317,6 +317,11 @@
     if hasattr(L, "am355_resident_counters"):
         L.am355_resident_counters.argtypes = [vp, vp]
         L.am355_resident_counters.restype = ctypes.c_int
+    if hasattr(L, "am355_device_span_counters"):
+        L.am355_device_span_counters.argtypes = [vp, vp]
+        L.am355_device_span_counters.restype = ctypes.c_int
+        L.am355_test_spans.argtypes = [vp, vp, vp, u32, vp, vp, u32, ctypes.POINTER(u32), ctypes.POINTER(u32)]
+        L.am355_test_spans.restype = ctypes.c_int
     if hasattr(L, "am355_resident_maps_only_calls"):
         L.am355_resident_maps_only_calls.argtypes = [vp, ctypes.POINTER(ctypes.c_uint64)]
         L.am355_resident_maps_only_calls.restype = ctypes.c_int
@@ -866,6 +871,22 @@
         self._check(self._L.am355_resident_counters(self._h, out))
         return int(out[0]), int(out[1]), int(out[2])
 
+    def device_span_counters(self):
+        out = (ctypes.c_uint64 * 3)()
+        self._check(self._L.am355_device_span_counters(self._h, out))
+        return int(out[0]), int(out[1]), int(out[2])
+
+    def test_spans(self):
+        ns, nt = ctypes.c_uint32(), ctypes.c_uint32()
+        rc = self._L.am355_test_spans(self._h, None, None, 0, None, None, 0, ctypes.byref(ns), ctypes.byref(nt))
+        if rc != AM355_E_ARG:
+            self._check(rc)
+        n, t = int(ns.value), int(nt.value)
+        ds, hs = np.zeros((n, 3), dtype=np.uint32), np.zeros((n, 3), dtype=np.uint32)
+        dt, ht = np.zeros(t, dtype=np.uint32), np.zeros(t, dtype=np.uint32)
+        self._check(self._L.am355_test_spans(self._h, ds.ctypes.data, hs.ctypes.data, n, dt.ctypes.data, ht.ctypes.data, t, ctypes.byref(ns), ctypes.byref(nt)))
+        return ds, hs, dt, ht
+
     def resident_maps_only_calls(self):
         out = ctypes.c_uint64()
         self._check(self._L.am355_resident_maps_only_calls(self._h, ctypes.byref(out)))
diff --git a/include/am355.h b/include/am355.h
--- a/include/am355.h
+++ b/include/am355.h
@@ -199,6 +199,9 @@
 
 int am355_resident_counters(const am355_ctx *ctx, uint64_t out[3]);
 int am355_resident_maps_only_calls(const am355_ctx *ctx, uint64_t *out);
+int am355_device_span_counters(const am355_ctx *ctx, uint64_t out[3]);
+int am355_test_spans(am355_ctx *ctx, uint32_t *dev_spans, uint32_t *host_spans, uint32_t cap_spans, uint32_t *dev_tab, uint32_t *host_tab,
+                     uint32_t cap_tab, uint32_t *n_spans, uint32_t *n_tab);
 int am355_set_resident_new_actors(am355_ctx *ctx, int on);
 int am355_resident_new_actor_calls(const am355_ctx *ctx, uint64_t out[2]);
 int am355_set_resident_map_merge(am355_ctx *ctx, int on);
```

New measurement: 1.126 billion. 0.915x the previous value.
